# plurigrid/moose

Measured on AMD Instinct MI355X. Metric: replicated fixed(14,23) matmul elems/sec, higher is better.
Workload: dtype fixed(14,23) over Z_2^128 (exact multi-modular int8-MFMA GEMM)

## Files before the change

csrc/gemm_crt.hip:

```cpp
#include <hip/hip_runtime.h>

#include <algorithm>
#include <cmath>
#include <cstdint>
#include <cstdlib>
#include <cstring>
#include <mutex>

#include "hip_attr.h"
#include "moosex.h"
#include "prf_dev.h"
#include "rss_fused.h"

void mx_ws_note(int dev, int64_t want, bool ok);
bool mx_ws_malloc(void** p, int64_t bytes);
void mx_ws_shared_note(void);

namespace {

using u64 = uint64_t;
using u128 = unsigned __int128;
typedef int v4i __attribute__((ext_vector_type(4)));
typedef int v16i __attribute__((ext_vector_type(16)));

// ... 997 lines not shown
      r = r == STG - 1 ? 0 : r + 1;
    }
  }
  asm volatile("s_waitcnt vmcnt(0)" ::: "memory");

  const float pf = ep.pf[mi], rcp = ep.rcp[mi];
  const int t16 = ep.t16[mi];
  int8_t* cr = CR + ((int64_t)g * ntiles + tm * tiles_n + tn) * (int64_t)(BM * BN);
#pragma unroll
  for (int i = 0; i < MI; ++i)
#pragma unroll
    for (int j = 0; j < NJ; ++j) {
      int rr[4];
#pragma unroll
      for (int e = 0; e < 4; ++e)
        rr[e] = centered_mod(acc[i][j][e], pf, rcp, t16);
      const int bi = wr * MI + i, bj = wc * NJ + j;
      *(uint32_t*)(cr + ((bi * (BN / 16) + bj) * 64 + lane) * 4) = pack4(rr[0], rr[1], rr[2], rr[3]);
    }
}

template <class T, int BN>
__global__ void __launch_bounds__(256)
    k_crt_recon16(const int8_t* __restrict__ CR, T* __restrict__ C, int64_t M, int64_t N,
                  int64_t tiles_m, int64_t tiles_n, int accumulate, const RecTab rc) {
  constexpr int NK = sizeof(T) / 2;
  constexpr int kCrTile = BM * BN, NBJ = BN / 16;
  const int64_t ntiles = tiles_m * tiles_n;
  const int64_t total = ntiles * (kCrTile / 4);
  const int64_t b = blockIdx.y;
  const int n = rc.n;
  for (int64_t gt = blockIdx.x * (int64_t)blockDim.x + threadIdx.x; gt < total;
       gt += (int64_t)gridDim.x * blockDim.x) {
    const int lane = (int)(gt & 63);
    const int64_t rest = gt >> 6;
    const int blk = (int)(rest % (16 * NBJ));
    const int64_t tile = rest / (16 * NBJ);
    const int64_t off = tile * kCrTile + (blk * 64 + lane) * 4;
    int acc[4][NK];
    float qs[4];
#pragma unroll
    for (int e = 0; e < 4; ++e) {
      qs[e] = 0.f;
#pragma unroll
      for (int k = 0; k < NK; ++k) acc[e][k] = 0;
    }
    const int8_t* src = CR + b * n * ntiles * (int64_t)kCrTile + off;
    for (int i = 0; i < n; ++i) {
      const uint32_t v = *(const uint32_t*)(src + i * ntiles * (int64_t)kCrTile);
      const float rcp = rc.rcp[i];
      int wk[NK];
#pragma unroll
      for (int k = 0; k < NK; ++k) wk[k] = rc.W[i][k];
#pragma unroll
      for (int e = 0; e < 4; ++e) {
        const int c = (int)(int8_t)((v >> (8 * e)) & 0xff);
        qs[e] = __builtin_fmaf((float)c, rcp, qs[e]);
#pragma unroll
        for (int k = 0; k < NK; ++k) acc[e][k] += __mul24(c, wk[k]);
      }
    }
    const int64_t tm = tile / tiles_n, tn = tile % tiles_n;
    const int bi = blk / NBJ, bj = blk % NBJ;
    const int64_t gcol = tn * BN + bj * 16 + (lane & 15);
    T mw = 0;
#pragma unroll
    for (int k = 0; k < NK; ++k) mw |= (T)rc.Mw[k] << (16 * k);
#pragma unroll
    for (int e = 0; e < 4; ++e) {
      const int64_t grow = tm * BM + bi * 16 + 4 * (lane >> 4) + e;
      T z = 0;
#pragma unroll
      for (int k = 0; k < NK; ++k) z += (T)(int64_t)acc[e][k] << (16 * k);
      const int q = (int)__builtin_rintf(qs[e]);
      z -= (T)(int64_t)q * mw;
      if (grow < M && gcol < N) {
        T* pc = C + (b * M + grow) * N + gcol;
        *pc = accumulate ? (T)(*pc + z) : z;
      }
    }
  }
}

template <class T, int BN>
__global__ void __launch_bounds__(256)
    k_crt_recon16d(const int8_t* __restrict__ CR, T* __restrict__ C, int64_t M, int64_t N,
                   int64_t tiles_m, int64_t tiles_n, int accumulate, const RecTab4 r4, int n,
                   const RecTab rc) {
  constexpr int ND = (int)sizeof(T);
  constexpr int NK = ND / 2;
  constexpr int kCrTile = BM * BN, NBJ = BN / 16;
  const int64_t ntiles = tiles_m * tiles_n;
  const int64_t total = ntiles * (kCrTile / 4);
  const int64_t b = blockIdx.y;
  for (int64_t gt = blockIdx.x * (int64_t)blockDim.x + threadIdx.x; gt < total;
       gt += (int64_t)gridDim.x * blockDim.x) {
    const int lane = (int)(gt & 63);
    const int64_t rest = gt >> 6;
    const int blk = (int)(rest % (16 * NBJ));
    const int64_t tile = rest / (16 * NBJ);
    const int64_t off = tile * kCrTile + (blk * 64 + lane) * 4;
    int acc[4][ND], aq[4][3];
#pragma unroll
    for (int e = 0; e < 4; ++e) {
#pragma unroll
      for (int d = 0; d < ND; ++d) acc[e][d] = 0;
#pragma unroll
      for (int d = 0; d < 3; ++d) aq[e][d] = 0;
    }
    const int8_t* src = CR + b * n * ntiles * (int64_t)kCrTile + off;
    const int64_t pstride = ntiles * (int64_t)kCrTile;
    for (int g = 0; g < r4.groups; ++g) {
      uint32_t v[4];
#pragma unroll
      for (int u = 0; u < 4; ++u)
        v[u] = 4 * g + u < n ? *(const uint32_t*)(src + (4 * g + u) * pstride) : 0u;
      const uint32_t a0 = __builtin_amdgcn_perm(v[1], v[0], 0x05010400u);
      const uint32_t a1 = __builtin_amdgcn_perm(v[1], v[0], 0x07030602u);
      const uint32_t c0 = __builtin_amdgcn_perm(v[3], v[2], 0x05010400u);
      const uint32_t c1 = __builtin_amdgcn_perm(v[3], v[2], 0x07030602u);
      const int t[4] = {(int)__builtin_amdgcn_perm(c0, a0, 0x05040100u),
                        (int)__builtin_amdgcn_perm(c0, a0, 0x07060302u),
                        (int)__builtin_amdgcn_perm(c1, a1, 0x05040100u),
                        (int)__builtin_amdgcn_perm(c1, a1, 0x07060302u)};
#pragma unroll
      for (int d = 0; d < ND; ++d) {
        const int w = (int)r4.wd[g][d];
#pragma unroll
        for (int e = 0; e < 4; ++e) acc[e][d] = __builtin_amdgcn_sdot4(t[e], w, acc[e][d], false);
      }
#pragma unroll
      for (int d = 0; d < 3; ++d) {
        const int w = (int)r4.rd[g][d];
#pragma unroll
        for (int e = 0; e < 4; ++e) aq[e][d] = __builtin_amdgcn_sdot4(t[e], w, aq[e][d], false);
      }
    }
    const int64_t tm = tile / tiles_n, tn = tile % tiles_n;
    const int bi = blk / NBJ, bj = blk % NBJ;
    const int64_t gcol = tn * BN + bj * 16 + (lane & 15);
    T mw = 0;
#pragma unroll
    for (int k = 0; k < NK; ++k) mw |= (T)rc.Mw[k] << (16 * k);
#pragma unroll
    for (int e = 0; e < 4; ++e) {
      const int64_t grow = tm * BM + bi * 16 + 4 * (lane >> 4) + e;
      T z = 0;
#pragma unroll
      for (int k = 0; k < NK; ++k)
        z += (T)(int64_t)(acc[e][2 * k] + acc[e][2 * k + 1] * 256) << (16 * k);
      const int64_t F = (int64_t)aq[e][0] + (int64_t)aq[e][1] * 256 + (int64_t)aq[e][2] * 65536;
      const int64_t q = (F + (1 << 23)) >> 24;
      z -= (T)q * mw;
      if (grow < M && gcol < N) {
        T* pc = C + (b * M + grow) * N + gcol;
        *pc = accumulate ? (T)(*pc + z) : z;
      }
    }
  }
}

inline int64_t round_up(int64_t x, int64_t m) { return (x + m - 1) / m * m; }

int crt_kernel() {
  const char* e = std::getenv("MOOSEX_CRT_KERNEL");
  const int v = e ? std::atoi(e) : 8;
  return v >= 1 && v <= 16 ? v : 8;
}
bool crt_mfma16() { return crt_kernel() >= 4; }
int recon_dot4() {
  static const int v = [] {
    const char* e = std::getenv("MOOSEX_CRT_RECON");
    return e && e[0] == '0' ? 0 : 1;
  }();
  return v;
}

struct CPlan {
  int n, bn;
  int64_t tiles_m, tiles_n, nkb, a_nkb, ra_bytes, rb_bytes, cr_bytes;
};

CPlan make_cplan(int words, int64_t batch, int64_t M, int64_t N, int64_t K, int mode,
                 bool roll = false) {
  CPlan p;
  p.bn = (crt_kernel() == 3 || crt_kernel() == 5) ? 128 : 256;
  const int64_t kprime = mode ? 2 * K : K;
  p.n = moduli_needed(words, kprime);
  p.tiles_m = (M + BM - 1) / BM;
  p.tiles_n = (N + p.bn - 1) / p.bn;
  p.nkb = round_up(kprime, BK) / BK;
  p.a_nkb = roll ? p.nkb / 2 : p.nkb;
  p.ra_bytes = batch * p.n * p.tiles_m * p.a_nkb * (int64_t)kImg;
  p.rb_bytes = batch * p.n * p.tiles_n * p.nkb * (int64_t)(p.bn * BK);
  p.cr_bytes = batch * p.n * p.tiles_m * p.tiles_n * (int64_t)(BM * p.bn);
  return p;
}

int gemm_group_m() {
  const char* e = std::getenv("MOOSEX_CRT_GROUPM");
  const int v = e ? std::atoi(e) : 8;
  return v >= 1 && v <= 64 ? v : 8;
}

bool prep_packed() {
  static const bool v = [] {
    const char* e = std::getenv("MOOSEX_CRT_PACKED");
    return !(e && e[0] == '0');
  }();
  return v;
}

template <class T>
void launch_prep(const CPlan& p, const Tables& tb, bool is_b, int64_t batch, int64_t R,
                 int64_t K, int64_t xs, const T* X0, const T* X1, int mode, int8_t* out,
                 hipStream_t st, int64_t nkb = -1, int64_t nkb_s = -1,
                 const PrepSrcs& src = PrepSrcs()) {
  if (nkb < 0) nkb = p.nkb;
  if (nkb_s < nkb) nkb_s = nkb;
  const int64_t tiles = is_b ? p.tiles_n : p.tiles_m;
  const int rows = is_b ? p.bn : BM;
  const int64_t work = tiles * nkb * (rows * 4);
  const dim3 grid((unsigned)std::min<int64_t>((work + 255) / 256, 16384), (unsigned)batch);
  static const bool packed_b = [] {
    const char* e = std::getenv("MOOSEX_CRT_PACKED_B");
    return e && e[0] == '1';
  }();
  if (!prep_packed() || (is_b && !packed_b)) {
    if (!is_b)
      hipLaunchKernelGGL((k_crt_prep<T, false, BM, false>), grid, dim3(256), 0, st, X0, X1, R, K,
                         xs, mode, out, tiles, nkb, nkb_s, tb.pa, src);
    else if (rows == 256)
      hipLaunchKernelGGL((k_crt_prep<T, true, 256, false>), grid, dim3(256), 0, st, X0, X1, R, K,
                         xs, mode, out, tiles, nkb, nkb_s, tb.pb, src);
    else
      hipLaunchKernelGGL((k_crt_prep<T, true, 128, false>), grid, dim3(256), 0, st, X0, X1, R, K,
                         xs, mode, out, tiles, nkb, nkb_s, tb.pb, src);
    return;
  }
  if (!is_b)
    hipLaunchKernelGGL((k_crt_prep<T, false, BM>), grid, dim3(256), 0, st, X0, X1, R, K, xs, mode,
// ... 51 lines not shown
    hipLaunchKernelGGL((k_crt_prep_src<true, 256, false>), grid, dim3(256), 0, st, s, src.key, R,
                       K, out, tiles, p.a_nkb, tb.pb);
  else
    hipLaunchKernelGGL((k_crt_prep_src<true, 128, false>), grid, dim3(256), 0, st, s, src.key, R,
                       K, out, tiles, p.a_nkb, tb.pb);
}

int dma_mask() {
  const char* e = std::getenv("MOOSEX_CRT_DMA_MASK");
  return e ? std::atoi(e) : 3;
}

template <int WR, int WC, int BN, int MINW, bool M16, int STG = kStages, int IL = 0>
void launch_variant(const CPlan& p, const Tables& tb, int64_t batch, const int8_t* ra,
                    const int8_t* rb, int8_t* cr, int bcast, int roll, hipStream_t st,
                    int amap = 0, int bmap = 0) {
  constexpr int lds = STG * (kImg + BN * BK);
  const void* fn = M16 ? (const void*)k_crt_gemm16<WR, WC, BN, MINW, STG, IL>
                       : (const void*)k_crt_gemm<WR, WC, BN, MINW>;
  ensure_lds_attr(fn, lds, st);
  const dim3 grid((unsigned)(p.tiles_m * p.tiles_n), (unsigned)(batch * p.n));
  if constexpr (M16)
    hipLaunchKernelGGL((k_crt_gemm16<WR, WC, BN, MINW, STG, IL>), grid, dim3(64 * WR * WC), lds, st, ra,
                       rb, cr, (int)p.tiles_m, (int)p.tiles_n, (int)p.nkb, gemm_group_m(), tb.ep,
                       dma_mask(), bcast, (int)p.a_nkb, roll, amap, bmap);
  else
    hipLaunchKernelGGL((k_crt_gemm<WR, WC, BN, MINW>), grid, dim3(64 * WR * WC), lds, st, ra, rb,
                       cr, (int)p.tiles_m, (int)p.tiles_n, (int)p.nkb, gemm_group_m(), tb.ep,
                       dma_mask(), bcast);
}

void launch_crt_gemm(const CPlan& p, const Tables& tb, int64_t batch, const int8_t* ra,
                     const int8_t* rb, int8_t* cr, int bcast, int roll, hipStream_t st,
                     int amap = 0, int bmap = 0) {
  switch (crt_kernel()) {
    case 1: launch_variant<2, 2, 256, 1, false>(p, tb, batch, ra, rb, cr, bcast, 0, st); break;
    case 2: launch_variant<2, 4, 256, 2, false>(p, tb, batch, ra, rb, cr, bcast, 0, st); break;
    case 4: launch_variant<2, 2, 256, 1, true>(p, tb, batch, ra, rb, cr, bcast, roll, st, amap, bmap); break;
    case 3: launch_variant<2, 2, 128, 2, false>(p, tb, batch, ra, rb, cr, bcast, 0, st); break;
    case 6: launch_variant<2, 4, 256, 2, true>(p, tb, batch, ra, rb, cr, bcast, roll, st, amap, bmap); break;
    case 7: launch_variant<2, 4, 256, 2, true, 4>(p, tb, batch, ra, rb, cr, bcast, roll, st, amap, bmap); break;
    case 8: launch_variant<2, 4, 256, 2, true, 3, 1>(p, tb, batch, ra, rb, cr, bcast, roll, st, amap, bmap); break;
    case 9: launch_variant<2, 4, 256, 2, true, 4, 1>(p, tb, batch, ra, rb, cr, bcast, roll, st, amap, bmap); break;
    case 10: launch_variant<2, 4, 256, 2, true, 3, 2>(p, tb, batch, ra, rb, cr, bcast, roll, st, amap, bmap); break;
    case 11: launch_variant<2, 4, 256, 2, true, 4, 2>(p, tb, batch, ra, rb, cr, bcast, roll, st, amap, bmap); break;
    case 12: launch_variant<2, 2, 256, 1, true, 3, 1>(p, tb, batch, ra, rb, cr, bcast, roll, st, amap, bmap); break;
    case 13: launch_variant<2, 2, 256, 1, true, 4, 1>(p, tb, batch, ra, rb, cr, bcast, roll, st, amap, bmap); break;
    case 14: launch_variant<2, 2, 256, 1, true, 3, 2>(p, tb, batch, ra, rb, cr, bcast, roll, st, amap, bmap); break;
    case 15: launch_variant<2, 2, 256, 1, true, 4, 2>(p, tb, batch, ra, rb, cr, bcast, roll, st, amap, bmap); break;
    case 16: launch_variant<2, 4, 256, 2, true, 5, 3>(p, tb, batch, ra, rb, cr, bcast, roll, st, amap, bmap); break;
    default: launch_variant<2, 2, 128, 2, true>(p, tb, batch, ra, rb, cr, bcast, roll, st, amap, bmap); break;
  }
}

template <class T>
void launch_recon(const CPlan& p, const Tables& tb, int64_t batch, int64_t M, int64_t N,
                  const int8_t* cr, T* C, int accumulate, hipStream_t st) {
  const int64_t work = p.tiles_m * p.tiles_n * (BM * p.bn / 8);
  const int gx = (int)std::min<int64_t>((work + 255) / 256, 16384);
  if (crt_mfma16() && recon_dot4()) {
    const int gx16 = (int)std::min<int64_t>((2 * work + 255) / 256, 16384);
    if (p.bn == 256)
      hipLaunchKernelGGL((k_crt_recon16d<T, 256>), dim3(gx16, (unsigned)batch), dim3(256), 0, st,
                         cr, C, M, N, p.tiles_m, p.tiles_n, accumulate, tb.r4, p.n, tb.rc);
    else
      hipLaunchKernelGGL((k_crt_recon16d<T, 128>), dim3(gx16, (unsigned)batch), dim3(256), 0, st,
                         cr, C, M, N, p.tiles_m, p.tiles_n, accumulate, tb.r4, p.n, tb.rc);
  } else if (crt_mfma16()) {
    const int gx16 = (int)std::min<int64_t>((2 * work + 255) / 256, 16384);
    if (p.bn == 256)
      hipLaunchKernelGGL((k_crt_recon16<T, 256>), dim3(gx16, (unsigned)batch), dim3(256), 0, st,
                         cr, C, M, N, p.tiles_m, p.tiles_n, accumulate, tb.rc);
    else
      hipLaunchKernelGGL((k_crt_recon16<T, 128>), dim3(gx16, (unsigned)batch), dim3(256), 0, st,
                         cr, C, M, N, p.tiles_m, p.tiles_n, accumulate, tb.rc);
  } else if (p.bn == 256)
    hipLaunchKernelGGL((k_crt_recon<T, 256>), dim3(gx, (unsigned)batch), dim3(256), 0, st, cr, C,
                       M, N, p.tiles_m, p.tiles_n, accumulate, tb.rc);
  else
    hipLaunchKernelGGL((k_crt_recon<T, 128>), dim3(gx, (unsigned)batch), dim3(256), 0, st, cr, C,
                       M, N, p.tiles_m, p.tiles_n, accumulate, tb.rc);
}

struct Ws {
  void* ptr = nullptr;
  int64_t bytes = 0;
  hipStream_t stream = nullptr;
  bool used = false;
};
std::mutex g_mu;
constexpr int kWsPerDev = 128;
Ws g_ws[16][kWsPerDev];

void* workspace(int64_t bytes, hipStream_t st) {
  int dev = 0;
  hipGetDevice(&dev);
  if (dev < 0 || dev >= 16) return nullptr;
  std::lock_guard<std::mutex> lk(g_mu);
  Ws* slot = nullptr;
  for (int i = 0; i < kWsPerDev && !slot; ++i)
    if (g_ws[dev][i].used && g_ws[dev][i].stream == st) slot = &g_ws[dev][i];
  for (int i = 0; i < kWsPerDev && !slot; ++i)
    if (!g_ws[dev][i].used) {
      slot = &g_ws[dev][i];
      slot->used = true;
      slot->stream = st;
    }
  if (!slot) {
    slot = &g_ws[dev][kWsPerDev - 1];
    mx_ws_shared_note();
  }
  Ws& w = *slot;
  if (w.bytes < bytes) {
    int64_t want = 1 << 20;
    while (want < bytes) want <<= 1;
    void* q = nullptr;
    const bool ok = mx_ws_malloc(&q, want);
    mx_ws_note(dev, want, ok);
    if (!ok) return nullptr;
    w.ptr = q;
    w.bytes = want;
  }
  return w.ptr;
}

template <class T>
int run_crt(int64_t batch, int64_t M, int64_t N, int64_t K, const T* A0, const T* A1,
            int64_t a_bstride, const T* B0, const T* B1, int64_t b_bstride,
            const int8_t* rb_pre, int mode, T* C, int accumulate, hipStream_t st,
            int64_t roll = 0) {
  constexpr int words = sizeof(T) / 8;
  if (roll && (mode != 1 || K % BK || !crt_mfma16() || a_bstride == 0 || batch < 2 ||
               roll % batch == 0))
    return -7;
  const CPlan p = make_cplan(words, batch, M, N, K, mode, roll != 0);
  if (p.n < 0) return -6;
  if ((mode ? 2 * K : K) > (1 << 15)) return -6;
  const Tables& tb = tables_for(words, p.n);
  const int64_t need = p.ra_bytes + (rb_pre ? 0 : p.rb_bytes) + p.cr_bytes;
  int8_t* ws = (int8_t*)workspace(need, st);
  if (!ws) return -4;
  int8_t* ra = ws;
  int8_t* cr = ra + p.ra_bytes;
  const int8_t* rb = rb_pre;
  const bool a_bc = batch > 1 && a_bstride == 0;
  const bool b_bc = batch > 1 && b_bstride == 0 && !rb_pre;
  if (!rb) {
    int8_t* rbw = cr + p.cr_bytes;
    launch_prep<T>(p, tb, true, b_bc ? 1 : batch, N, K, b_bstride, B0, B1, mode, rbw, st);
    rb = rbw;
  }
  if (roll)
    launch_prep<T>(p, tb, false, batch, M, K, a_bstride, A0, A0, 0, ra, st, p.a_nkb);
  else
    launch_prep<T>(p, tb, false, a_bc ? 1 : batch, M, K, a_bstride, A0, A1, mode, ra, st);
  launch_crt_gemm(p, tb, batch, ra, rb, cr, (a_bc ? 1 : 0) | (b_bc ? 2 : 0),
                  (int)(((roll % batch) + batch) % batch), st);
  launch_recon<T>(p, tb, batch, M, N, cr, C, accumulate, st);
  const hipError_t e = hipGetLastError();
  return e != hipSuccess ? -100 - (int)e : 0;
}

template <class T>
int run_crt_asym(int64_t M, int64_t N, int64_t K, const T* S0, const T* S1, const T* T0,
                 const T* T1, int rolled, T* C, hipStream_t st, const ShareSrc* xs = nullptr,
                 const ShareSrc* ys = nullptr) {
  constexpr int words = sizeof(T) / 8;
  if (K % BK || !crt_mfma16()) return -7;
  if (2 * K > (1 << 15)) return -6;
  const CPlan p = make_cplan(words, 3, M, N, K, 1, true);
  if (p.n < 0) return -6;
  const Tables& tb = tables_for(words, p.n);
  const int64_t sa = M * K, sb = K * N;
  const T* a[3];
  const T* b[3];
  const T* c[3];
  const T* d[3];
  for (int q = 0; q < 3; ++q) {
    a[q] = S0 + q * sa;
    b[q] = rolled ? S0 + ((q + 1) % 3) * sa : S1 + q * sa;
    c[q] = T0 + q * sb;
    d[q] = rolled ? T0 + ((q + 1) % 3) * sb : T1 + q * sb;
  }
  int na, nb, amap, bmap;
  const int64_t a_entry = p.n * p.tiles_m * p.a_nkb * (int64_t)kImg;
  const int64_t b_entry = p.n * p.tiles_n * p.a_nkb * (int64_t)(p.bn * BK);
  auto pmap = [](int e0, int e1, int e2, int e3, int e4) {
    return (int)(0x80000000u | (unsigned)e0 | (1u << 6) | ((unsigned)(e1 | (e2 << 3)) << 8) |
                 ((unsigned)(e3 | (e4 << 3)) << 16));
  };
  if (rolled) {
    na = 4;
    nb = 4;
    amap = pmap(0, 1, 2, 1, 3);
    bmap = pmap(0, 1, 2, 3, 2);
  } else {
    na = 5;
    nb = 5;
    amap = pmap(0, 1, 2, 3, 4);
    bmap = pmap(0, 1, 2, 3, 4);
  }
  static const bool asum = [] {
    const char* e = std::getenv("MOOSEX_CRT_ASUM");
    return !(e && e[0] == '0');
  }();
  static const bool dual = [] {
    const char* e = std::getenv("MOOSEX_CRT_DUAL");
    return !(e && e[0] == '0');
  }();
  const bool duals = rolled && dual;
  if (xs || ys) {
    if (words != 2 || !duals) return -7;
    if (xs && (K % 256 || !share_src_ok(*xs))) return -7;
    if (ys && (N % 256 || !share_src_ok(*ys))) return -7;
  }
  static const bool zstrip = [] {
    const char* e = std::getenv("MOOSEX_ZERO_STRIP");
    return !(e && e[0] == '0');
  }();
  int aph[4], bph[4], aat[4] = {0, 1, 2, 3}, bat[4] = {0, 1, 2, 3};
  int64_t a_strip = 0, b_strip = 0;
  auto plan_src = [&](bool is_b, const ShareSrc& s, int (&ph)[4], int (&at)[4], int& n, int& map,
                      int64_t& strip) {
    src_phases(is_b, s, ph);
    int m = 0;
    for (int e = 0; e < 4; ++e) at[e] = zstrip && ph[e] == 3 ? kZeroStrip : m++;
    if (m == n) return;
    n = m;
    strip = p.a_nkb * (int64_t)(is_b ? p.bn * BK : kImg);
    for (int sh : {0, 8, 11, 16, 19}) map = (map & ~(7 << sh)) | (at[(map >> sh) & 7] << sh);
  };
  if (xs) plan_src(false, *xs, aph, aat, na, amap, a_strip);
  if (ys) plan_src(true, *ys, bph, bat, nb, bmap, b_strip);
  const int64_t ra_bytes = na * a_entry, rb_bytes = nb * b_entry;
  const int64_t sum_bytes = asum && !duals ? round_up(sa * (int64_t)sizeof(T), 256) : 0;
  int8_t* ws = (int8_t*)workspace(
      a_strip + ra_bytes + p.cr_bytes + b_strip + rb_bytes + sum_bytes, st);
  if (!ws) return -4;
  int8_t* ra = ws + a_strip;
  int8_t* cr = ra + ra_bytes;
  int8_t* rb = cr + p.cr_bytes + b_strip;
  T* a01 = sum_bytes ? (T*)(rb + rb_bytes) : nullptr;
  if (a01)
    hipLaunchKernelGGL((k_add_pair<T>), dim3((unsigned)std::min<int64_t>((sa + 255) / 256, 65536)),
                       dim3(256), 0, st, a[0], b[0], a01, sa);
  const int64_t kn = p.a_nkb;
  PrepSrcs sa_, sb_;
  auto put = [](PrepSrcs& q, const T* x0, const T* x1, int mode, int64_t dual = 0) {
    q.x0[q.n] = x0;
    q.x1[q.n] = x1;
    q.mode[q.n] = mode;
    q.dual[q.n] = dual;
    ++q.n;
  };
  if (duals) {
    put(sa_, a[2], a[2], 0);
    put(sa_, a[1], a[1], 0);
    put(sa_, a[0], b[0], 0, -3 * a_entry);
    put(sb_, d[1], c[1], 0, -b_entry);
    put(sb_, d[2], d[0], 0, -3 * b_entry);
    if (ys)
      launch_prep_src(p, tb, true, *ys, N, K, rb, b_entry, bph, bat, -b_strip, st);
    else
      launch_prep<T>(p, tb, true, sb_.n, N, K, 0, nullptr, nullptr, 0, rb + 2 * b_entry, st, kn,
                     kn, sb_);
    if (xs)
      launch_prep_src(p, tb, false, *xs, M, K, ra, a_entry, aph, aat, -a_strip, st);
    else
      launch_prep<T>(p, tb, false, sa_.n, M, K, 0, nullptr, nullptr, 0, ra + a_entry, st, kn, kn,
                     sa_);
  } else {
    if (a01)
      put(sa_, a01, a01, 0);
    else
      put(sa_, a[0], b[0], 2);
    put(sb_, c[0], d[0], 3);
    put(sb_, c[1], d[1], 3);
    if (rolled) {
      for (const T* e : {a[2], a[1], a[0]}) put(sa_, e, e, 0);
      for (const T* f : {d[1], d[2]}) put(sb_, f, f, 0);
    } else {
      for (const T* e : {b[1], a[1], a[2], b[2]}) put(sa_, e, e, 0);
      for (const T* f : {d[1], d[2], c[2]}) put(sb_, f, f, 0);
    }
    launch_prep<T>(p, tb, true, sb_.n, N, K, 0, nullptr, nullptr, 0, rb, st, kn, kn, sb_);
    launch_prep<T>(p, tb, false, sa_.n, M, K, 0, nullptr, nullptr, 0, ra, st, kn, kn, sa_);
  }
  launch_crt_gemm(p, tb, 3, ra, rb, cr, 0, 0, st, amap, bmap);
  launch_recon<T>(p, tb, 3, M, N, cr, C, 0, st);
  const hipError_t e = hipGetLastError();
  return e != hipSuccess ? -100 - (int)e : 0;
}

}

extern "C" {

int mx_gemm_asym(int words, int64_t M, int64_t N, int64_t K, const void* S0, const void* S1,
                 const void* T0, const void* T1, int rolled, void* C, void* stream) {
  if (M == 0 || N == 0) return 0;
  if (!rolled && (!S1 || !T1)) return -2;
  hipStream_t st = (hipStream_t)stream;
  if (words == 1)
    return run_crt_asym<u64>(M, N, K, (const u64*)S0, (const u64*)S1, (const u64*)T0,
                             (const u64*)T1, rolled, (u64*)C, st);
  if (words == 2)
    return run_crt_asym<u128>(M, N, K, (const u128*)S0, (const u128*)S1, (const u128*)T0,
                              (const u128*)T1, rolled, (u128*)C, st);
  return -2;
}

int mx_gemm_asym_src(int words, int64_t M, int64_t N, int64_t K, const void* S0, const void* T0,
                     const int64_t* xsrc, const int64_t* ysrc, void* C, void* stream) {
  if (M == 0 || N == 0) return 0;
  if (words != 2) return -7;
  if ((!xsrc && !S0) || (!ysrc && !T0)) return -2;
  ShareSrc sx, sy;
  auto fill = [](ShareSrc& s, const int64_t* a) {
    s.x = (const void*)(intptr_t)a[0];
    s.kind = (int)a[1];
    s.frac = (int)a[2];
    s.j0 = (int)a[3];
    const uint32_t* slot[1] = {(const uint32_t*)(intptr_t)a[4]};
    s.key = mxd::keysrc_slots(slot, 1);
    s.nonce = (uint64_t)a[5];
  };
  if (xsrc) fill(sx, xsrc);
  if (ysrc) fill(sy, ysrc);
  if ((xsrc && !sx.key.slot[0]) || (ysrc && !sy.key.slot[0])) return -2;
  return run_crt_asym<u128>(M, N, K, (const u128*)S0, nullptr, (const u128*)T0, nullptr, 1,
                            (u128*)C, (hipStream_t)stream, xsrc ? &sx : nullptr,
                            ysrc ? &sy : nullptr);
}

int mx_crt_moduli(int words, int64_t kprime) {
  if (words != 1 && words != 2) return -2;
  return moduli_needed(words, kprime);
}

int mx_crt_tables(int words, int n, int32_t* p_out, uint8_t* wa_out, uint8_t* wb_out,
                  int32_t* nega_out, int32_t* negb_out, uint16_t* W_out, uint16_t* Mw_out) {
  if ((words != 1 && words != 2) || n < 1 || n > kMaxMod) return -2;
  const Tables& t = tables_for(words, n);
  for (int i = 0; i < n; ++i) {
    p_out[i] = t.ep.p[i];
    for (int j = 0; j < 16; ++j) {
      wa_out[i * 16 + j] = (uint8_t)(t.pa.w[i][j / 4] >> (8 * (j % 4)));
      wb_out[i * 16 + j] = (uint8_t)(t.pb.w[i][j / 4] >> (8 * (j % 4)));
    }
    nega_out[i] = (int32_t)t.pa.neg[i];
    negb_out[i] = (int32_t)t.pb.neg[i];
    if (i == 0) {
      nega_out[0] = (int32_t)t.pa.mul0;
      negb_out[0] = 1;
    }
    for (int k = 0; k < 8; ++k) W_out[i * 8 + k] = t.rc.W[i][k];
  }
  for (int k = 0; k < 8; ++k) Mw_out[k] = t.rc.Mw[k];
  return 0;
}

int mx_crt_tables4(int words, int n, uint32_t* wd_out, uint32_t* rd_out) {
  if ((words != 1 && words != 2) || n < 1 || n > kMaxMod) return -2;
  const Tables& t = tables_for(words, n);
  for (int g = 0; g < t.r4.groups; ++g) {
    for (int d = 0; d < 16; ++d) wd_out[g * 16 + d] = t.r4.wd[g][d];
    for (int d = 0; d < 3; ++d) rd_out[g * 3 + d] = t.r4.rd[g][d];
  }
  return t.r4.groups;
}

int mx_crt_combine(int words, int n, int side, int i, int64_t count, const int32_t* ra,
                   const int32_t* rb, const int32_t* kappa, int8_t* out) {
  if ((words != 1 && words != 2) || n < 1 || n > kMaxMod || i < 0 || i >= n || (side & ~1))
    return -2;
  const Tables& t = tables_for(words, n);
  const PrepTab& tab = side ? t.pb : t.pa;
  const float p = (float)tab.p[i], rcp = tab.rcp[i];
  for (int64_t k = 0; k < count; ++k) {
    if (side) {
      out[k] = (int8_t)crt_combine(ra[k], rb[k], kappa[k], tab.neg[i], p, rcp);
    } else {
      const f2 f = crt_combine2((f2){(float)ra[k], 0.f}, (f2){(float)rb[k], 0.f},
                                (f2){(float)kappa[k], 0.f}, (float)tab.neg[i], p, rcp);
      out[k] = (int8_t)(int)f.x;
    }
  }
  return 0;
}

int mxh_gemm_crt(int words, int64_t batch, int64_t M, int64_t N, int64_t K, const void* A0,
                 const void* A1, const void* B0, const void* B1, int mode, void* C,
                 int accumulate, void* stream) {
  hipStream_t st = (hipStream_t)stream;
  if (words == 1)
    return run_crt<u64>(batch, M, N, K, (const u64*)A0, (const u64*)A1, M * K, (const u64*)B0,
                        (const u64*)B1, K * N, nullptr, mode, (u64*)C, accumulate, st);
  if (words == 2)
    return run_crt<u128>(batch, M, N, K, (const u128*)A0, (const u128*)A1, M * K,
                         (const u128*)B0, (const u128*)B1, K * N, nullptr, mode, (u128*)C,
                         accumulate, st);
  return -2;
}

int mxh_gemm_crt_strided(int words, int64_t batch, int64_t M, int64_t N, int64_t K,
                         const void* A0, const void* A1, int64_t a_bstride, const void* B0,
                         const void* B1, int64_t b_bstride, int mode, void* C, int accumulate,
                         void* stream) {
  hipStream_t st = (hipStream_t)stream;
  if (words == 1)
    return run_crt<u64>(batch, M, N, K, (const u64*)A0, (const u64*)A1, a_bstride,
                        (const u64*)B0, (const u64*)B1, b_bstride, nullptr, mode, (u64*)C,
                        accumulate, st);
  if (words == 2)
    return run_crt<u128>(batch, M, N, K, (const u128*)A0, (const u128*)A1, a_bstride,
// ... 59 lines not shown
```

csrc/moosex.h:

```cpp
#pragma once
#include <stdint.h>

#ifdef __cplusplus
extern "C" {
#endif

enum mx_binop { MX_ADD = 0, MX_SUB = 1, MX_MUL = 2, MX_AND = 3, MX_OR = 4, MX_XOR = 5 };
enum mx_unop { MX_NEG = 0, MX_NOT = 1, MX_SHL = 2, MX_SHR = 3, MX_SAR = 4 };
enum mx_cmpop { MX_LT = 0, MX_GT = 1, MX_EQ = 2, MX_MSB = 3 };
enum mx_cross { MX_CROSS_ARITH = 0, MX_CROSS_BOOL = 1 };
enum mx_share_src { MX_SHARE_F64 = 2, MX_SHARE_MIRROR = 8 };

typedef struct {
  uint32_t rk[44];
} mx_aes_key;

int mx_version(void);
int mx_device_count(void);

int mx_ew_binary(int dev, int op, int words, const void* a, int64_t na, const void* b,
                 int64_t nb, void* out, int64_t n, void* stream);
int mx_ew_binary_slot(int dev, int op, int words, const void* a, const void* b, int64_t nb,
                      void* out, int64_t m, int nparties, int which, void* stream);
int mx_add_zs3(int dev, int words, const void* v, const void* r, void* out0, void* out1,
               int64_t n, void* stream);
int mx_ew_unary(int dev, int op, int words, const void* a, void* out, int64_t n,
                int64_t param, void* stream);
int mx_ew_binary2(int dev, int op, int words, const void* a0, const void* b0, void* out0,
                  const void* a1, const void* b1, void* out1, int64_t na, int64_t nb, int64_t n,
                  void* stream);
int mx_mul_add2(int dev, int words, const void* a0, const void* a1, const void* f,
                const void* c, int add0, int add1, void* out0, void* out1, int64_t n,
                void* stream);
int mx_ew_unary2(int dev, int op, int words, const void* a0, void* out0, const void* a1,
                 void* out1, int64_t n, int64_t param, void* stream);
int mx_transpose2(int dev, int words, const void* a0, void* out0, const void* a1, void* out1,
                  int64_t rows, int64_t cols, void* stream);
int mx_im2col(int dev, int elem_bytes, const void* in, void* out, int64_t slots,
              int64_t in_slot_stride, int64_t N, int64_t C, int64_t H, int64_t W, int64_t KH,
              int64_t KW, int64_t sh, int64_t sw, int64_t pt, int64_t pl, int64_t dh,
              int64_t dw, int64_t OH, int64_t OW, int nhwc, void* stream);
int mx_col2im(int dev, int elem_bytes, const void* in, void* out, int64_t slots,
              int64_t in_slot_stride, int64_t N, int64_t C, int64_t H, int64_t W, int64_t KH,
              int64_t KW, int64_t sh, int64_t sw, int64_t pt, int64_t pl, int64_t dh,
              int64_t dw, int64_t OH, int64_t OW, int nhwc, void* stream);
int mx_resize2d(int dev, int elem_bytes, const void* in, void* out, int64_t slots,
                int64_t in_slot_stride, int64_t N, int64_t C, int64_t H, int64_t W, int64_t OH,
                int64_t OW, const int32_t* th, const int32_t* tw, int wbh, int wbw, int nhwc,
                void* stream);
int mx_dwconv(int dev, int elem_bytes, const void* x0, const void* x1, const void* w0,
              const void* w1, void* out, int64_t slots, int64_t x_slot_stride,
              int64_t w_slot_stride, int64_t N, int64_t C, int64_t H, int64_t W, int64_t mult,
              int64_t KH, int64_t KW, int64_t sh, int64_t sw, int64_t pt, int64_t pl,
              int64_t dh, int64_t dw, int64_t OH, int64_t OW, int nhwc, void* stream);
#define MX_PWL_MAX 8
int mx_pwl_cross(int dev, int elem_bytes, const void* s0, const void* s1, const void* x0,
                 const void* x1, void* out, int64_t slots, int64_t s_slot_stride,
                 int64_t x_slot_stride, int64_t n, int k, const uint64_t* da, const uint64_t* db,
                 const uint64_t* ak, void* stream);
int mx_ew_binary_slot2(int dev, int op, int words, const void* a0, const void* a1,
                       const void* b, int64_t nb, void* out0, void* out1, int64_t m,
                       int nparties, int which0, int which1, void* stream);
int mx_mul_trunc3_kv(int dev, int words, const void* x0, const void* x1, const void* y0,
                     const void* y1, void* out0, void* out1, int64_t n, int64_t ostride,
                     const uint32_t* slots, uint64_t nmul, int m, const uint64_t* nonces,
                     const int64_t* views, void* stream);
int mx_mul_trunc3_open(int dev, int words, const void* x, int64_t xstride, double* out,
                       int64_t n, const uint32_t* slots, uint64_t nmul, int m,
                       const uint64_t* nonces, int frac, void* stream);
int mx_ew_add3(int dev, int words, const void* a, const void* b, const void* c, void* out,
               int64_t n, void* stream);
int mx_lincomb2(int dev, int words, int nin, const void* const* ins, const int64_t* coef,
                const void* b, int64_t nb, void* out0, void* out1, int64_t m, int nparties,
                int which0, int which1, void* stream);
int mx_sum_views2(int dev, int words, const void* base0, const void* base1, int64_t is0,
                  int64_t is1, int64_t ps0, int64_t ps1, int k, void* out0, void* out1, int64_t m,
                  int nparties, void* stream);
int mx_slot_place2(int dev, int words, const void* x0, const void* x1, void* out0, void* out1,
                   int64_t m, int nparties, int which0, int which1, void* stream);
int mx_ew_compare(int dev, int op, int words, const void* a, int64_t na, const void* b,
                  int64_t nb, uint8_t* out, int64_t n, void* stream);
int mx_bit_extract(int dev, int words, const void* a, uint8_t* out, int64_t n, int bit,
                   void* stream);
int mx_ring_inject(int dev, int words, const uint8_t* bits, void* out, int64_t n, int bit,
                   void* stream);
int mx_encode(int dev, int words, const double* x, void* out, int64_t n, int frac,
              void* stream);
int mx_addn_decode(int dev, int words, const void* a, const void* b, const void* c,
                   const void* d, double* out, int64_t n, int frac, void* stream);
int mx_decode(int dev, int words, const void* x, double* out, int64_t n, int frac,
              void* stream);
int mx_fill(int dev, int words, void* out, int64_t n, uint64_t lo, uint64_t hi, void* stream);
int mx_bit_planes(int dev, int words, const void* a, uint8_t* out, int64_t outer, int64_t inner,
                  int start, int count, void* stream);
int mx_weighted_sum(int dev, int words, const void* a, const void* w, void* out, int64_t outer,
                    int64_t k, int64_t inner, void* stream);
int mx_sum_axis(int dev, int words, const void* a, void* out, int64_t outer, int64_t red,
                int64_t inner, void* stream);
int mx_prg(int dev, const uint8_t* key16, uint64_t nonce, uint64_t ctr0, void* out,
           int64_t nbytes, void* stream);
int mx_derive_seed(const uint8_t* key16, const uint8_t* sync16, uint8_t* out16);
int mx_aes_encrypt_blocks(const uint8_t* key16, const uint8_t* in, uint8_t* out,
                          int64_t nblocks);
int mx_rss_cross(int dev, int kind, int words, const void* x0, const void* x1,
                 const void* y0, const void* y1, void* out, int64_t n, int nparties,
                 const uint8_t* keys16, uint64_t nonce, void* stream);
int mx_zero_share(int dev, int kind, int words, void* out, int64_t n, int nparties,
                  const uint8_t* keys16, uint64_t nonce, void* stream);
int mx_prf_expand(int dev, int words, void* out, int64_t n, int nkeys,
                  const uint8_t* keys16, uint64_t nonce, void* stream);
int mx_gemm(int dev, int words, int64_t batch, int64_t M, int64_t N, int64_t K,
            const void* A0, const void* A1, const void* B0, const void* B1, int mode,
            void* C, int accumulate, void* stream);
int64_t mx_gemm_workspace_bytes(int words, int64_t batch, int64_t M, int64_t N,
                                int64_t K, int mode);
int64_t mx_workspace_failed_bytes(void);
int64_t mx_workspace_held_bytes(void);
int64_t mx_workspace_shared_count(void);
int mx_gemm_ws(int words, int64_t batch, int64_t M, int64_t N, int64_t K, const void* A0,
               const void* A1, const void* B0, const void* B1, int mode, void* C,
               int accumulate, void* workspace, int64_t ws_bytes, void* stream);
int64_t mx_gemm_b_bytes(int words, int64_t batch, int64_t N, int64_t K, int mode);
int mx_gemm_prep_b(int words, int64_t batch, int64_t K, int64_t N, const void* B0,
                   const void* B1, int mode, void* lb, void* stream);
int mx_gemm_with_b(int words, int64_t batch, int64_t M, int64_t N, int64_t K, const void* A0,
                   const void* A1, int64_t a_bstride, int mode, const void* lb, void* C,
                   int accumulate, void* stream);
int mx_crt_tables4(int words, int n, uint32_t* wd_out, uint32_t* rd_out);
int mx_gemm_roll(int words, int64_t batch, int64_t M, int64_t N, int64_t K, const void* A0,
                 int64_t a_bstride, int64_t roll, const void* B0, const void* B1, const void* lb,
                 void* C, int accumulate, void* stream);
int mx_gemm_strided(int words, int64_t batch, int64_t M, int64_t N, int64_t K, const void* A0,
                    const void* A1, int64_t a_bstride, const void* B0, const void* B1,
                    int64_t b_bstride, int mode, void* C, int accumulate, void* stream);
void mx_set_gemm_impl(int impl);
void mx_set_gemm_crt(int mode);
int mx_crt_moduli(int words, int64_t kprime);
int mx_crt_tables(int words, int n, int32_t* p, uint8_t* wa, uint8_t* wb, int32_t* nega,
                  int32_t* negb, uint16_t* W, uint16_t* Mw);
int mx_crt_combine(int words, int n, int side, int i, int64_t count, const int32_t* ra,
                   const int32_t* rb, const int32_t* kappa, int8_t* out);

int mx_trunc_pr3(int dev, int words, const void* s0, void* out0, void* out1, int64_t n, int m,
                 const uint8_t* k0, const uint8_t* k2, const uint64_t* nonces, void* stream);
int mx_share3(int dev, int kind, int words, const void* x, void* out0, void* out1, int64_t n,
              int j, const uint8_t* k_next, const uint8_t* k_all, uint64_t n1, uint64_t na,
              void* stream);

#define MX_KEY_SLOT_WORDS 48
void mx_key_slots(const uint8_t* keys16, int n, uint32_t* out);
int mx_rss_cross_k(int dev, int kind, int words, const void* x0, const void* x1,
                   const void* y0, const void* y1, void* out, int64_t n, int nparties,
// ... 112 lines not shown
```

csrc/ring_common.h:

```cpp
#pragma once
#include <stdint.h>
#include <string.h>

#include "aes_core.h"
#include "img_geom.h"
#include "moosex.h"

namespace mxr {

using u64 = uint64_t;
using u128 = unsigned __int128;
using i128 = __int128;

template <class T>
struct Bits {
  static constexpr int value = 8 * sizeof(T);
};

template <class T>
MX_HD inline T binop(int op, T a, T b) {
  if constexpr (sizeof(T) == 1) {
    switch (op) {
      case MX_ADD:
      case MX_SUB:
// ... 64 lines not shown
    }
  } else {
    i128 x = (i128)a, y = (i128)b;
    switch (op) {
      case MX_LT: return x < y;
      case MX_GT: return x > y;
      case MX_EQ: return x == y;
      default: return (uint8_t)(a >> 127);
    }
  }
}

template <class T>
MX_HD inline T cross(int kind, T x0, T x1, T y0, T y1, bool has_x1, bool has_y1) {
  if (kind == MX_CROSS_BOOL) {
    T v = x0 & y0;
    if (has_y1) v ^= x0 & y1;
    if (has_x1) v ^= x1 & y0;
    return v;
  }
  T v = x0 * y0;
  if (has_y1) v += x0 * y1;
  if (has_x1) v += x1 * y0;
  return v;
}

template <class T>
MX_HD inline T zs_combine(int kind, T v, T ra, T rb) {
  if (kind == MX_CROSS_BOOL) return (T)(v ^ ra ^ rb);
  return (T)(v + ra - rb);
}


MX_HD inline i128 f64_to_i128(double x) {
  uint64_t bits;
  memcpy(&bits, &x, 8);
  int neg = (int)(bits >> 63);
  int e = (int)((bits >> 52) & 0x7ff);
  uint64_t mant = bits & ((1ull << 52) - 1);
  if (e == 0x7ff) return mant ? (i128)0 : (neg ? (i128)((u128)1 << 127) : ~(i128)((u128)1 << 127));
  if (e == 0) return 0;
  mant |= (1ull << 52);
  int sh = e - 1075;
  u128 mag;
  if (sh >= 0) {
    if (sh > 127 - 53) return neg ? (i128)((u128)1 << 127) : ~(i128)((u128)1 << 127);
    mag = (u128)mant << sh;
  } else if (sh <= -53) {
    mag = 0;
  } else {
    mag = (u128)(mant >> (-sh));
  }
  return neg ? -(i128)mag : (i128)mag;
}

template <class T>
MX_HD inline T f64_to_ring(double x) {
  if constexpr (sizeof(T) == 8) {
    if (x >= 9223372036854775808.0) return (T)0x7fffffffffffffffull;
    if (x > -9223372036854775808.0) return (T)(int64_t)x;
    return x != x ? (T)0 : (T)1 << 63;
  } else {
    return (T)f64_to_i128(x);
  }
}

MX_HD inline double i128_to_f64(u128 v) {
  const bool neg = (v >> 127) != 0;
  const u128 m = neg ? (u128)0 - v : v;
  const uint64_t hi = (uint64_t)(m >> 64), lo = (uint64_t)m;
  double r;
  if (hi == 0) {
    r = (double)lo;
  } else {
    const int s = 64 - __builtin_clzll(hi);
    const uint64_t lost = s == 64 ? lo : lo & ((1ull << s) - 1);
    const uint64_t top = (uint64_t)(m >> s) | (uint64_t)(lost != 0);
    const uint64_t pbits = (uint64_t)(1023 + s) << 52;
    double p;
    memcpy(&p, &pbits, 8);
    r = (double)top * p;
  }
  return neg ? -r : r;
}

}

extern "C" {
int mxh_ew_binary(int op, int words, const void* a, int64_t na, const void* b, int64_t nb,
                  void* out, int64_t n, void* stream);
int mxh_ew_unary(int op, int words, const void* a, void* out, int64_t n, int64_t param,
                 void* stream);
int mxh_ew_compare(int op, int words, const void* a, int64_t na, const void* b, int64_t nb,
                   uint8_t* out, int64_t n, void* stream);
int mxh_bit_extract(int words, const void* a, uint8_t* out, int64_t n, int bit, void* stream);
int mxh_ring_inject(int words, const uint8_t* bits, void* out, int64_t n, int bit,
                    void* stream);
int mxh_encode(int words, const double* x, void* out, int64_t n, int frac, void* stream);
int mxh_decode(int words, const void* x, double* out, int64_t n, int frac, void* stream);
int mxh_addn_decode(int words, const void* a, const void* b, const void* c, const void* d,
                    double* out, int64_t n, int frac, void* stream);
int mxh_fill(int words, void* out, int64_t n, uint64_t lo, uint64_t hi, void* stream);
int mxh_bit_planes(int words, const void* a, uint8_t* out, int64_t outer, int64_t inner,
                   int start, int count, void* stream);
int mxh_weighted_sum(int words, const void* a, const void* w, void* out, int64_t outer,
                     int64_t k, int64_t inner, void* stream);
int mxh_sum_axis(int words, const void* a, void* out, int64_t outer, int64_t red, int64_t inner,
                 void* stream);
int mxh_prg(const uint8_t* key16, uint64_t nonce, uint64_t ctr0, void* out, int64_t nbytes,
            void* stream);
int mxh_rss_cross(int kind, int words, const void* x0, const void* x1, const void* y0,
                  const void* y1, void* out, int64_t n, int nparties, const uint8_t* keys16,
                  uint64_t nonce, void* stream);
int mxh_prf_expand(int words, void* out, int64_t n, int nkeys, const uint8_t* keys16,
                   uint64_t nonce, void* stream);
int mxh_rss_cross_kp(int kind, int words, const void* x0, const void* x1, const void* y0,
                     const void* y1, void* out, int64_t n, int nparties,
                     const uint32_t* const* slot_ptrs, uint64_t nonce, void* stream);
int mxh_rss_cross_k(int kind, int words, const void* x0, const void* x1, const void* y0,
                    const void* y1, void* out, int64_t n, int nparties, const uint32_t* slots,
                    int nslots, uint64_t nonce, void* stream);
int mxh_rss_mul3_kv(int kind, int words, const void* x0, const void* x1, const void* y0,
                    const void* y1, void* out0, void* out1, int64_t n, const uint32_t* slots,
                    uint64_t nonce, const int64_t* views, void* stream);
int mxh_rss_mul3_k(int kind, int words, const void* x0, const void* x1, const void* y0,
                   const void* y1, void* out0, void* out1, int64_t n, const uint32_t* slots,
                   uint64_t nonce, void* stream);
int mxh_ew_binary_slot(int op, int words, const void* a, const void* b, int64_t nb, void* out,
                       int64_t m, int nparties, int which, void* stream);
int mxh_add_zs3(int words, const void* v, const void* r, void* out0, void* out1, int64_t n,
                void* stream);
int mxh_ew_binary2(int op, int words, const void* a0, const void* b0, void* out0,
                   const void* a1, const void* b1, void* out1, int64_t na, int64_t nb, int64_t n,
                   void* stream);
int mxh_mul_add2(int words, const void* a0, const void* a1, const void* f, const void* c,
                 int add0, int add1, void* out0, void* out1, int64_t n, void* stream);
int mxh_ew_add3(int words, const void* a, const void* b, const void* c, void* out, int64_t n,
                void* stream);
int mxh_lincomb2(int words, int nin, const void* const* ins, const int64_t* coef, const void* b,
                 int64_t nb, void* out0, void* out1, int64_t m, int nparties, int which0,
                 int which1, void* stream);
int mxh_sum_views2(int words, const void* base0, const void* base1, int64_t is0, int64_t is1,
                   int64_t ps0, int64_t ps1, int k, void* out0, void* out1, int64_t m,
                   int nparties, void* stream);
int mxh_slot_place2(int words, const void* x0, const void* x1, void* out0, void* out1,
                    int64_t m, int nparties, int which0, int which1, void* stream);
int mxh_mul_trunc3_kv(int words, const void* x0, const void* x1, const void* y0, const void* y1,
                      void* out0, void* out1, int64_t n, int64_t ostride, const uint32_t* slots,
                      uint64_t nmul, int m, const uint64_t* nn, const int64_t* views,
                      void* stream);
int mxh_mul_trunc3_open(int words, const void* x, int64_t xstride, double* out, int64_t n,
                        const uint32_t* slots, uint64_t nmul, int m, const uint64_t* nn, int frac,
                        void* stream);
int mxh_ew_unary2(int op, int words, const void* a0, void* out0, const void* a1, void* out1,
                  int64_t n, int64_t param, void* stream);
int mxh_transpose2(int words, const void* a0, void* out0, const void* a1, void* out1,
                   int64_t rows, int64_t cols, void* stream);
int mxh_ew_binary_slot2(int op, int words, const void* a0, const void* a1, const void* b,
                        int64_t nb, void* out0, void* out1, int64_t m, int nparties, int which0,
                        int which1, void* stream);
int mxh_im2col(int elem_bytes, const void* in, void* out, int64_t slots, int64_t in_slot_stride,
               const mxr::ImgGeom& g, void* stream);
int mxh_col2im(int elem_bytes, const void* in, void* out, int64_t slots, int64_t in_slot_stride,
               const mxr::ImgGeom& g, void* stream);
int mxh_resize2d(int elem_bytes, const void* in, void* out, int64_t slots,
                 int64_t in_slot_stride, const mxr::ImgGeom& g, const int32_t* th,
                 const int32_t* tw, void* stream);
int mxh_pwl_cross(int elem_bytes, const void* s0, const void* s1, const void* x0, const void* x1,
                  void* out, int64_t slots, int64_t s_slot_stride, int64_t x_slot_stride,
                  int64_t n, int k, const uint64_t* da, const uint64_t* db, const uint64_t* ak,
                  void* stream);
int mxh_dwconv(int elem_bytes, const void* x0, const void* x1, const void* w0, const void* w1,
               void* out, int64_t slots, int64_t x_slot_stride, int64_t w_slot_stride,
               const mxr::ImgGeom& g, void* stream);
int mxh_ks_cross1(int words, const void* g0, const void* g1, const void* p0, const void* p1,
                  void* z, int64_t n, int d, int both, const uint8_t* keys16, uint64_t nonce,
                  void* stream);
int mxh_ks_cross1_s(int words, const void* g0, const void* g1, const void* p0, const void* p1,
                    void* z, int64_t n, int d, int both, const uint32_t* const* slots,
                    uint64_t nonce, void* stream);
int mxh_ks_cross1x_s(int words, const void* g0, const void* g1, const void* t0, const void* t1,
                     void* go0, void* go1, const void* p0, const void* p1, void* z, int64_t n,
                     int d, int both, const uint32_t* const* slots, uint64_t nonce,
                     void* stream);
int mxh_ks_sum2(int words, const void* p0, const void* p1, const void* g0, const void* g1,
                const void* t0, const void* t1, void* o0, void* o1, int64_t n, void* stream);
int mxh_ks_adder3_k(int words, const void* g0, const void* g1, const void* p0, const void* p1,
                    void* og0, void* og1, int64_t n, int nlev, const uint32_t* slots,
                    const uint64_t* nonces, void* stream);
int mxh_ks_level3_k(int words, const void* g0, const void* g1, const void* p0, const void* p1,
                    void* og0, void* og1, void* op0, void* op1, int64_t n, int d, int both,
                    const uint32_t* slots, uint64_t nonce, void* stream);
int mxh_prf_expand_k(int words, void* out, int64_t n, int nkeys, const uint32_t* slots,
                     uint64_t nonce, void* stream);
int mxh_gemm(int words, int64_t batch, int64_t M, int64_t N, int64_t K, const void* A0,
             const void* A1, const void* B0, const void* B1, int mode, void* C, int accumulate,
             void* stream);
}
```

csrc/ring_hip.hip:

```cpp
#include <hip/hip_runtime.h>

#include <algorithm>
#include <cstring>
#include <type_traits>

#include "prf_dev.h"
#include "moosex.h"
#include "party_batch.h"
#include "ring_common.h"
#include "rss_fused.h"

using mxr::u128;
using u64 = uint64_t;

namespace {

constexpr int kBlock = 256;

inline int grid_for(int64_t n, int per_thread = 1) {
  int64_t blocks = (n + (int64_t)kBlock * per_thread - 1) / ((int64_t)kBlock * per_thread);
  return (int)std::max<int64_t>(1, std::min<int64_t>(blocks, 256 * 8));
}

inline hipStream_t S(void* s) { return (hipStream_t)s; }
// ... 1308 lines not shown
                                                             const T* __restrict__ y0,
                                                             const T* __restrict__ y1,
                                                             T* __restrict__ out,
                                                             T* __restrict__ out1, int64_t n,
                                                             KeySrc keys, uint64_t nonce, Views vw) {
  constexpr int EPB = 256 / 3;
  __shared__ uint32_t rks[3][kKeyWords];
  __shared__ uint64_t kl[3][EPB], kh[3][EPB];
  stage_keys(rks, keys, 3);
  constexpr int P = Lane<T>::kPer;
  const int64_t nb = (n + P - 1) / P;
  const int tid = threadIdx.x, s = tid / EPB, lb = tid % EPB;
  for (int64_t b0 = (int64_t)blockIdx.x * EPB; b0 < nb; b0 += (int64_t)gridDim.x * EPB) {
    const bool fin = tid < EPB && b0 + tid < nb;
    T vv[3][P];
#pragma unroll
    for (int p = 0; p < 3; ++p) {
#pragma unroll
      for (int j = 0; j < P; ++j) {
        const int64_t e = (b0 + tid) * P + j;
        T v = 0;
        if (fin && e < n) {
          if (x0 != nullptr && y0 != nullptr)
            v = mxr::cross<T>(kind, ld_view(x0, vw, 0, p, e, n),
                              x1 ? ld_view(x1, vw, 1, p, e, n) : (T)0, ld_view(y0, vw, 2, p, e, n),
                              y1 ? ld_view(y1, vw, 3, p, e, n) : (T)0, x1 != nullptr, y1 != nullptr);
          else if (x0 != nullptr)
            v = ld_view(x0, vw, 0, p, e, n);
        }
        vv[p][j] = v;
      }
    }
    if (s < 3 && b0 + lb < nb) {
      uint64_t lo, hi;
      prf_chunk(rks[s], nonce, (uint64_t)(b0 + lb), &lo, &hi);
      kl[s][lb] = lo;
      kh[s][lb] = hi;
    }
    __syncthreads();
    if (fin) {
      const int64_t b = b0 + tid;
#pragma unroll
      for (int p = 0; p < 3; ++p) {
        const int q = p == 2 ? 0 : p + 1;
#pragma unroll
        for (int j = 0; j < P; ++j) {
          const int64_t e = b * P + j;
          if (e >= n) break;
          const int64_t i = (int64_t)p * n + e;
          const T v = vv[p][j];
          const T z = mxr::zs_combine<T>(kind, v, pick<T>(kl[p][tid], kh[p][tid], j),
                                         pick<T>(kl[q][tid], kh[q][tid], j));
          out[i] = z;
          if (out1 != nullptr) out1[(int64_t)(p == 0 ? 2 : p - 1) * n + e] = z;
        }
      }
    }
    __syncthreads();
  }
}

template <class T>
struct TailShares {
  T* __restrict__ out0;
  T* __restrict__ out1;
  int64_t os;
  __device__ __forceinline__ void operator()(int64_t e, T Z0, T Z1, T Z2) const {
    out0[e] = Z0;
    out0[os + e] = Z1;
    out0[2 * os + e] = Z2;
    if (out1 != out0 + os) {
      out1[e] = Z1;
      out1[os + e] = Z2;
    }
    out1[2 * os + e] = Z0;
  }
};

template <class T>
struct TailOpen {
  double* __restrict__ out;
  double scale;
  __device__ __forceinline__ void operator()(int64_t e, T Z0, T Z1, T Z2) const {
    const T v = Z0 + Z1 + Z2;
    if constexpr (sizeof(T) == 8)
      out[e] = (double)(int64_t)v * scale;
    else
      out[e] = mxr::i128_to_f64(v) * scale;
  }
};

template <class T, int EPB, class Sink>
__device__ __forceinline__ void mul_trunc3_lat_body(
    const T* __restrict__ x0, const T* __restrict__ x1, const T* __restrict__ y0,
    const T* __restrict__ y1, const Sink& sink, int64_t n,
    const uint32_t (&rks)[3][kKeyWords], uint64_t (&kl)[9][EPB], uint64_t (&kh)[9][EPB],
    uint64_t nmul, int m, uint64_t nr0, uint64_t nr1, uint64_t nt, uint64_t nm, uint64_t nz0,
    uint64_t nz2, const Views& vw) {
  constexpr int NS = 9;
  constexpr int P = Lane<T>::kPer;
  const int64_t nb = (n + P - 1) / P;
  const int tid = threadIdx.x, s = tid / EPB, lb = tid % EPB;
  const int key_of = s < 3 ? s : (s == 4 || s == 8) ? 2 : 0;
  const uint64_t nonce_of = s < 3 ? nmul : s == 3 ? nr0 : s == 4 ? nr1 : s == 5 ? nt
                            : s == 6 ? nm : s == 7 ? nz0 : nz2;
  for (int64_t b0 = (int64_t)blockIdx.x * EPB; b0 < nb; b0 += (int64_t)gridDim.x * EPB) {
    const bool fin = tid < EPB && b0 + tid < nb;
    T vv[P][3];
#pragma unroll
    for (int j = 0; j < P; ++j) {
      const int64_t e = (b0 + tid) * P + j;
#pragma unroll
      for (int p = 0; p < 3; ++p)
        vv[j][p] = !fin || e >= n ? (T)0
                   : y0 == nullptr ? ld_view(x0, vw, 0, p, e, n)
                   : mxr::cross<T>(MX_CROSS_ARITH, ld_view(x0, vw, 0, p, e, n),
                                   ld_view(x1, vw, 1, p, e, n), ld_view(y0, vw, 2, p, e, n),
                                   ld_view(y1, vw, 3, p, e, n), true, true);
    }
    if (s < NS && b0 + lb < nb) {
      uint64_t lo, hi;
      prf_chunk(rks[key_of], nonce_of, (uint64_t)(b0 + lb), &lo, &hi);
      kl[s][lb] = lo;
      kh[s][lb] = hi;
    }
    __syncthreads();
    if (fin) {
      const int64_t b = b0 + tid;
#pragma unroll
      for (int j = 0; j < P; ++j) {
        const int64_t e = b * P + j;
        if (e >= n) break;
        T z[3];
#pragma unroll
        for (int p = 0; p < 3; ++p) {
          const int q = p == 2 ? 0 : p + 1;
          z[p] = mxr::zs_combine<T>(MX_CROSS_ARITH, vv[j][p], pick<T>(kl[p][tid], kh[p][tid], j),
                                    pick<T>(kl[q][tid], kh[q][tid], j));
        }
        const T Z0 = pick<T>(kl[7][tid], kh[7][tid], j);
        const T Z2 = pick<T>(kl[8][tid], kh[8][tid], j);
        const T Z1 = mxf::trunc_pr_z1<T>(
            z[0], z[1], z[2], pick<T>(kl[3][tid], kh[3][tid], j),
            pick<T>(kl[4][tid], kh[4][tid], j), pick<T>(kl[5][tid], kh[5][tid], j),
            pick<T>(kl[6][tid], kh[6][tid], j), Z0, Z2, m);
        sink(e, Z0, Z1, Z2);
      }
    }
    __syncthreads();
  }
}

template <class T>
__global__ void __launch_bounds__(256) k_mul_trunc3_lat(
    const T* __restrict__ x0, const T* __restrict__ x1, const T* __restrict__ y0,
    const T* __restrict__ y1, T* __restrict__ out0, T* __restrict__ out1, int64_t n, int64_t os,
    KeySrc keys, uint64_t nmul, int m, uint64_t nr0, uint64_t nr1, uint64_t nt, uint64_t nm,
    uint64_t nz0, uint64_t nz2, Views vw) {
  constexpr int EPB = 256 / 9;
  __shared__ uint32_t rks[3][kKeyWords];
  __shared__ uint64_t kl[9][EPB], kh[9][EPB];
  stage_keys(rks, keys, 3);
  mul_trunc3_lat_body<T, EPB>(x0, x1, y0, y1, TailShares<T>{out0, out1, os}, n, rks, kl, kh,
                              nmul, m, nr0, nr1, nt, nm, nz0, nz2, vw);
}

template <class T>
__global__ void __launch_bounds__(256) k_mul_trunc3_lat_open(
    const T* __restrict__ x, double* __restrict__ out, double scale, int64_t n, KeySrc keys,
    uint64_t nmul, int m, uint64_t nr0, uint64_t nr1, uint64_t nt, uint64_t nm, uint64_t nz0,
    uint64_t nz2, Views vw) {
// ... 1805 lines not shown
```

csrc/rss_fused.h:

```cpp
#pragma once
#include <stdint.h>

#include "aes_core.h"
#include "moosex.h"
#include "ring_common.h"

namespace mxf {

template <class T>
MX_HD inline T shl(T x, int k) {
  constexpr int W = 8 * sizeof(T);
  return k >= W ? (T)0 : (T)(x << k);
}
template <class T>
MX_HD inline T shr(T x, int k) {
  constexpr int W = 8 * sizeof(T);
  return k >= W ? (T)0 : (T)(x >> k);
}

template <class T>
MX_HD inline T trunc_pr_z1(T x0, T x1, T x2, T r0, T r1, T rt0, T rm0, T z0, T z2, int m) {
  constexpr int W = 8 * sizeof(T);
  const int k = W - 1;
  T r = r0 + r1;
  T r_msb = shr<T>(r, W - 1);
  T r_top = shr<T>(shl<T>(r, 1), m + 1);
  T rt1 = r_top - rt0;
  T rm1 = r_msb - rm0;
  T mk0 = x0 + x1 + shl<T>((T)1, k - 1) + r0;
  T mk1 = x2 + r1;
  T c = mk0 + mk1;
  T c_msb = shr<T>(c, W - 1);
  T c_top = shr<T>(shl<T>(c, 1), m + 1);
  T ov0 = rm0 - shl<T>(c_msb * rm0, 1) + c_msb;
  T y0 = shl<T>(ov0, k - m) - rt0 + c_top - shl<T>((T)1, k - 1 - m);
  T ov1 = rm1 - shl<T>(c_msb * rm1, 1);
  T y1 = shl<T>(ov1, k - m) - rt1;
  return (y0 - z0) + (y1 - z2);
}

template <class T>
MX_HD inline T share_plain(int kind, const void* xv, int64_t i, double scale) {
  return kind == MX_SHARE_F64 ? mxr::f64_to_ring<T>(((const double*)xv)[i] * scale)
                              : ((const T*)xv)[i];
}
template <class T>
MX_HD inline T share_masked(int kind, T x, T r) {
  return kind == MX_CROSS_BOOL ? (T)(x ^ r) : (T)(x - r);
}
MX_HD inline void share_place(int j0, bool mir, int* jr, int* jv) {
  *jr = mir ? (j0 + 1) % 3 : j0;
  *jv = mir ? j0 : (j0 + 1) % 3;
}
template <class T>
MX_HD inline void share_slots(int kind, T x, T r, int j0, bool mir, T (&slot)[3]) {
  const T v = share_masked<T>(kind, x, r);
  slot[j0] = mir ? v : r;
  slot[(j0 + 1) % 3] = mir ? r : v;
  slot[(j0 + 2) % 3] = 0;
}

using u128_t = unsigned __int128;

constexpr int64_t kRingExtendLatMax = 8192;

MX_HD inline void ring_extend_dealer(uint64_t r0, uint64_t r1, u128_t R0, uint64_t M0, u128_t* R1,
                                     uint64_t* M1) {
  const uint64_t r = r0 + r1;
  *R1 = (u128_t)r - R0;
  *M1 = (r >> 63) - M0;
}

MX_HD inline uint64_t ring_extend_mask0(uint64_t x0, uint64_t x1, uint64_t r0) {
  return x0 + x1 + ((uint64_t)1 << 62) + r0;
}

MX_HD inline u128_t ring_extend_y(uint64_t c, u128_t R, uint64_t M, bool first) {
  const uint64_t nc = 1 - (c >> 63);
  const u128_t y = ((u128_t)(uint64_t)(nc * M) << 64) - R;
  return first ? y + (u128_t)c - ((u128_t)1 << 62) : y;
}

MX_HD inline u128_t ring_extend_z1(uint64_t x0, uint64_t x1, uint64_t x2, uint64_t r0, uint64_t r1,
                                   u128_t R0, uint64_t M0, u128_t z0, u128_t z2) {
  u128_t R1;
  uint64_t M1;
  ring_extend_dealer(r0, r1, R0, M0, &R1, &M1);
  const uint64_t c = ring_extend_mask0(x0, x1, r0) + (x2 + r1);
  const u128_t y0 = ring_extend_y(c, R0, M0, true);
  const u128_t y1 = ring_extend_y(c, R1, M1, false);
  return (y0 - z0) + (y1 - z2);
}

}

namespace mxf {

template <class T>
MX_HD inline void trunc_dealer(T r0, T r1, T rt0, T rm0, int m, T* rt1, uint64_t* rm1) {
  constexpr int W = 8 * sizeof(T);
  const T r = r0 + r1;
  *rt1 = shr<T>(shl<T>(r, 1), m + 1) - rt0;
  *rm1 = (uint64_t)(shr<T>(r, W - 1) - rm0);
}

template <class T>
MX_HD inline T trunc_mask0(T x0, T x1, T r0) {
  constexpr int W = 8 * sizeof(T);
  return x0 + x1 + shl<T>((T)1, W - 2) + r0;
}

template <class T>
MX_HD inline T trunc_y(T c, T rt, T rm, int m, bool first) {
  constexpr int W = 8 * sizeof(T);
  const int k = W - 1;
  const T c_msb = shr<T>(c, W - 1);
  T ov = rm - shl<T>(c_msb * rm, 1);
  if (!first) return shl<T>(ov, k - m) - rt;
  ov = ov + c_msb;
  const T c_top = shr<T>(shl<T>(c, 1), m + 1);
  return shl<T>(ov, k - m) - rt + c_top - shl<T>((T)1, k - 1 - m);
// ... 52 lines not shown
```

csrc/rss_fused_cpu.cpp:

```cpp
#include <cmath>
#include <cstring>
#include <functional>
#include <vector>

#include "moosex.h"
#include "ring_common.h"
#include "rss_fused.h"

void mx_cpu_prf_range(const uint8_t* key, uint64_t nonce, int words, int64_t i0, int64_t n,
                      void* out);
void mx_cpu_parallel_for(int64_t n, int64_t grain,
                         const std::function<void(int64_t, int64_t)>& f);

extern "C" int mxh_trunc_pr3(int words, const void* s0, void* out0, void* out1, int64_t n, int m,
                             const uint8_t* k0, const uint8_t* k2, const uint64_t* nonces,
                             void* stream);
extern "C" int mxh_share3(int kind, int words, const void* x, void* out0, void* out1, int64_t n,
                          int j, const uint8_t* k_next, const uint8_t* k_all, uint64_t n1,
                          uint64_t na, void* stream);
extern "C" int mxh_trunc_pr3_k(int words, const void* s0, void* out0, void* out1, int64_t n,
                               int m, const uint32_t* slot_k0, const uint32_t* slot_k2,
                               const uint64_t* nonces, void* stream);
extern "C" int mxh_trunc_pr3_kmo(int words, const void* s0, void* out0, void* out1, int64_t n,
                                 int m, const uint32_t* slot_k0, const uint32_t* slot_k2,
// ... 144 lines not shown
                 const uint8_t* k0, const uint8_t* k2, const uint64_t* nonces, void* stream) {
  if (dev) return mxh_trunc_pr3(words, s0, out0, out1, n, m, k0, k2, nonces, stream);
  if (words == 1)
    return trunc3_host<uint64_t>((const uint64_t*)s0, (uint64_t*)out0, (uint64_t*)out1, n, m, k0,
                                 k2, nonces);
  if (words == 2)
    return trunc3_host<unsigned __int128>((const unsigned __int128*)s0, (unsigned __int128*)out0,
                                          (unsigned __int128*)out1, n, m, k0, k2, nonces);
  return -2;
}

int mx_share3(int dev, int kind, int words, const void* x, void* out0, void* out1, int64_t n,
              int j, const uint8_t* k_next, const uint8_t* k_all, uint64_t n1, uint64_t na,
              void* stream) {
  if (dev) return mxh_share3(kind, words, x, out0, out1, n, j, k_next, k_all, n1, na, stream);
  switch (words) {
    case 0:
      return share3_host<uint8_t>(kind, (const uint8_t*)x, (uint8_t*)out0, (uint8_t*)out1, n, j,
                                  k_next, k_all, n1, na);
    case 1:
      return share3_host<uint64_t>(kind, (const uint64_t*)x, (uint64_t*)out0, (uint64_t*)out1, n,
                                   j, k_next, k_all, n1, na);
    case 2:
      return share3_host<unsigned __int128>(kind, (const unsigned __int128*)x,
                                            (unsigned __int128*)out0, (unsigned __int128*)out1, n,
                                            j, k_next, k_all, n1, na);
  }
  return -2;
}

int mx_trunc_pr3_k(int dev, int words, const void* s0, void* out0, void* out1, int64_t n, int m,
                   const uint32_t* slot_k0, const uint32_t* slot_k2, const uint64_t* nonces,
                   void* stream) {
  if (dev)
    return mxh_trunc_pr3_k(words, s0, out0, out1, n, m, slot_k0, slot_k2, nonces, stream);
  return mx_trunc_pr3(0, words, s0, out0, out1, n, m, (const uint8_t*)slot_k0,
                      (const uint8_t*)slot_k2, nonces, stream);
}

int mx_trunc_pr3_ko(int dev, int words, const void* s0, void* out0, void* out1, int64_t n,
                    int m, const uint32_t* slot_k0, const uint32_t* slot_k2,
                    const uint64_t* nonces, int64_t ostride, void* stream) {
  if (dev)
    return mxh_trunc_pr3_ko(words, s0, out0, out1, n, m, slot_k0, slot_k2, nonces, ostride,
                            stream);
  if (words != 1 && words != 2) return -2;
  const size_t es = 8 * (size_t)words;
  std::vector<uint8_t> t0(3 * n * es), t1(3 * n * es);
  int rc = mx_trunc_pr3_k(0, words, s0, t0.data(), t1.data(), n, m, slot_k0, slot_k2, nonces,
                          stream);
  if (rc) return rc;
  for (int p = 0; p < 3; ++p) {
    std::memcpy((uint8_t*)out0 + p * ostride * es, t0.data() + p * n * es, n * es);
    std::memcpy((uint8_t*)out1 + p * ostride * es, t1.data() + p * n * es, n * es);
  }
  return 0;
}

int mx_trunc_pr3_kmo(int dev, int words, const void* s0, void* out0, void* out1, int64_t n,
                     int m, const uint32_t* slot_k0, const uint32_t* slot_k2,
                     const uint64_t* nonces, int64_t ostride, const uint64_t* cm, void* stream) {
  if (dev)
    return mxh_trunc_pr3_kmo(words, s0, out0, out1, n, m, slot_k0, slot_k2, nonces, ostride, cm,
                             stream);
  if (words == 1) {
    std::vector<uint64_t> t(3 * n);
    for (int64_t i = 0; i < 3 * n; ++i) t[i] = ((const uint64_t*)s0)[i] * cm[0];
    return mx_trunc_pr3_ko(0, words, t.data(), out0, out1, n, m, slot_k0, slot_k2, nonces,
                           ostride, stream);
  }
  if (words == 2) {
    using u128 = unsigned __int128;
    const u128 c = ((u128)cm[1] << 64) | cm[0];
    std::vector<u128> t(3 * n);
    for (int64_t i = 0; i < 3 * n; ++i) t[i] = ((const u128*)s0)[i] * c;
    return mx_trunc_pr3_ko(0, words, t.data(), out0, out1, n, m, slot_k0, slot_k2, nonces,
                           ostride, stream);
  }
  return -2;
}

int mx_mul_trunc3_open(int dev, int words, const void* x, int64_t xstride, double* out,
                       int64_t n, const uint32_t* slots, uint64_t nmul, int m,
                       const uint64_t* nonces, int frac, void* stream) {
  if (words != 1 && words != 2) return -2;
  if (m < 1 || m > 63) return -3;
  if (dev) return mxh_mul_trunc3_open(words, x, xstride, out, n, slots, nmul, m, nonces, frac,
                                      stream);
  if (xstride < n) return -3;
  const uint8_t* k[3];
  for (int i = 0; i < 3; ++i) k[i] = (const uint8_t*)(slots + MX_KEY_SLOT_WORDS * i);
  if (words == 1)
    return mul_trunc3_open_host<uint64_t>((const uint64_t*)x, xstride, out, n, k, nmul, m,
                                          nonces, frac);
  return mul_trunc3_open_host<unsigned __int128>((const unsigned __int128*)x, xstride, out, n, k,
                                                 nmul, m, nonces, frac);
}

int mx_ring_extend3_k(int dev, const void* s0, void* out0, void* out1, int64_t n,
                      const uint32_t* slot_k0, const uint32_t* slot_k2, const uint64_t* nonces,
                      void* stream) {
  if (dev) return mxh_ring_extend3_k(s0, out0, out1, n, slot_k0, slot_k2, nonces, stream);
  return ring_extend3_host((const uint64_t*)s0, (unsigned __int128*)out0,
                           (unsigned __int128*)out1, n, (const uint8_t*)slot_k0,
                           (const uint8_t*)slot_k2, nonces);
}

int64_t mx_ring_extend3_lat_max(void) { return mxf::kRingExtendLatMax; }

int mx_share3_k(int dev, int kind, int words, const void* x, void* out0, void* out1, int64_t n,
                int j, const uint32_t* slot_next, const uint32_t* slot_all, uint64_t n1,
                uint64_t na, void* stream) {
  if (dev)
    return mxh_share3_k(kind, words, x, out0, out1, n, j, slot_next, slot_all, n1, na, stream);
  return mx_share3(0, kind, words, x, out0, out1, n, j, (const uint8_t*)slot_next,
                   (const uint8_t*)slot_all, n1, na, stream);
}

}
```

moose_amd/ops/native.py:

```python
from __future__ import annotations

import ctypes
import os
import threading

import torch

from moose_amd import errors
from moose_amd._native import build as _build

_LIB = None
_LOCK = threading.Lock()

c_i64 = ctypes.c_int64
c_int = ctypes.c_int
c_u64 = ctypes.c_uint64
c_vp = ctypes.c_void_p

_SIGS = {
    "mx_version": (c_int, []),
    "mx_device_count": (c_int, []),
    "mx_ew_binary": (c_int, [c_int, c_int, c_int, c_vp, c_i64, c_vp, c_i64, c_vp, c_i64, c_vp]),
    "mx_ew_unary": (c_int, [c_int, c_int, c_int, c_vp, c_vp, c_i64, c_i64, c_vp]),
    "mx_mul_add2": (c_int, [c_int, c_int, c_vp, c_vp, c_vp, c_vp, c_int, c_int, c_vp, c_vp,
                            c_i64, c_vp]),
    "mx_ew_binary2": (c_int, [c_int, c_int, c_int, c_vp, c_vp, c_vp, c_vp, c_vp, c_vp, c_i64,
                              c_i64, c_i64, c_vp]),
    "mx_ew_unary2": (c_int, [c_int, c_int, c_int, c_vp, c_vp, c_vp, c_vp, c_i64, c_i64, c_vp]),
    "mx_transpose2": (c_int, [c_int, c_int, c_vp, c_vp, c_vp, c_vp, c_i64, c_i64, c_vp]),
    "mx_im2col": (c_int, [c_int, c_int, c_vp, c_vp, c_i64, c_i64] + [c_i64] * 14 + [c_int, c_vp]),
    "mx_col2im": (c_int, [c_int, c_int, c_vp, c_vp, c_i64, c_i64] + [c_i64] * 14 + [c_int, c_vp]),
    "mx_resize2d": (c_int, [c_int, c_int, c_vp, c_vp, c_i64, c_i64] + [c_i64] * 6
                    + [c_vp, c_vp, c_int, c_int, c_int, c_vp]),
    "mx_pwl_cross": (c_int, [c_int, c_int] + [c_vp] * 5 + [c_i64] * 4 + [c_int] + [c_vp] * 3
                     + [c_vp]),
    "mx_dwconv": (c_int, [c_int, c_int] + [c_vp] * 5 + [c_i64] * 3 + [c_i64] * 15
                  + [c_int, c_vp]),
    "mx_ew_binary_slot2": (c_int, [c_int, c_int, c_int, c_vp, c_vp, c_vp, c_i64, c_vp, c_vp,
                                   c_i64, c_int, c_int, c_int, c_vp]),
    "mx_mul_trunc3_kv": (c_int, [c_int, c_int, c_vp, c_vp, c_vp, c_vp, c_vp, c_vp, c_i64, c_i64,
                                 c_vp, c_u64, c_int, c_vp, c_vp, c_vp]),
    "mx_mul_trunc3_open": (c_int, [c_int, c_int, c_vp, c_i64, c_vp, c_i64, c_vp, c_u64, c_int,
                                   c_vp, c_int, c_vp]),
    "mx_ew_add3": (c_int, [c_int, c_int, c_vp, c_vp, c_vp, c_vp, c_i64, c_vp]),
    "mx_lincomb2": (c_int, [c_int, c_int, c_int, c_vp, c_vp, c_vp, c_i64, c_vp, c_vp, c_i64,
                            c_int, c_int, c_int, c_vp]),
    "mx_sum_views2": (c_int, [c_int, c_int, c_vp, c_vp, c_i64, c_i64, c_i64, c_i64, c_int, c_vp,
                              c_vp, c_i64, c_int, c_vp]),
    "mx_slot_place2": (c_int, [c_int, c_int, c_vp, c_vp, c_vp, c_vp, c_i64, c_int, c_int, c_int,
                               c_vp]),
    "mx_ew_compare": (c_int, [c_int, c_int, c_int, c_vp, c_i64, c_vp, c_i64, c_vp, c_i64, c_vp]),
    "mx_bit_extract": (c_int, [c_int, c_int, c_vp, c_vp, c_i64, c_int, c_vp]),
    "mx_ring_inject": (c_int, [c_int, c_int, c_vp, c_vp, c_i64, c_int, c_vp]),
    "mx_encode": (c_int, [c_int, c_int, c_vp, c_vp, c_i64, c_int, c_vp]),
    "mx_decode": (c_int, [c_int, c_int, c_vp, c_vp, c_i64, c_int, c_vp]),
    "mx_addn_decode": (c_int, [c_int, c_int, c_vp, c_vp, c_vp, c_vp, c_vp, c_i64, c_int, c_vp]),
    "mx_sum_axis": (c_int, [c_int, c_int, c_vp, c_vp, c_i64, c_i64, c_i64, c_vp]),
    "mx_fill": (c_int, [c_int, c_int, c_vp, c_i64, c_u64, c_u64, c_vp]),
    "mx_bit_planes": (c_int, [c_int, c_int, c_vp, c_vp, c_i64, c_i64, c_int, c_int, c_vp]),
    "mx_weighted_sum": (c_int, [c_int, c_int, c_vp, c_vp, c_vp, c_i64, c_i64, c_i64, c_vp]),
    "mx_prg": (c_int, [c_int, c_vp, c_u64, c_u64, c_vp, c_i64, c_vp]),
    "mx_aes_encrypt_blocks": (c_int, [c_vp, c_vp, c_vp, c_i64]),
    "mx_derive_seed": (c_int, [c_vp, c_vp, c_vp]),
    "mx_rss_cross": (
        c_int,
        [c_int, c_int, c_int, c_vp, c_vp, c_vp, c_vp, c_vp, c_i64, c_int, c_vp, c_u64, c_vp],
    ),
    "mx_zero_share": (c_int, [c_int, c_int, c_int, c_vp, c_i64, c_int, c_vp, c_u64, c_vp]),
    "mx_prf_expand": (c_int, [c_int, c_int, c_vp, c_i64, c_int, c_vp, c_u64, c_vp]),
    "mx_gemm": (
        c_int,
        [c_int, c_int, c_i64, c_i64, c_i64, c_i64, c_vp, c_vp, c_vp, c_vp, c_int, c_vp, c_int, c_vp],
    ),
    "mx_gemm_workspace_bytes": (c_i64, [c_int, c_i64, c_i64, c_i64, c_i64, c_int]),
    "mx_workspace_failed_bytes": (c_i64, []),
    "mx_workspace_held_bytes": (c_i64, []),
    "mx_workspace_shared_count": (c_i64, []),
    "mx_mfma_peak": (c_int, [c_int, c_int, c_vp, c_vp]),
    "mx_gemm_ws": (
        c_int,
        [c_int, c_i64, c_i64, c_i64, c_i64, c_vp, c_vp, c_vp, c_vp, c_int, c_vp, c_int, c_vp,
         c_i64, c_vp],
    ),
    "mx_set_gemm_impl": (None, [c_int]),
    "mx_set_gemm_crt": (None, [c_int]),
    "mx_gemm_strided": (
        c_int,
        [c_int, c_i64, c_i64, c_i64, c_i64, c_vp, c_vp, c_i64, c_vp, c_vp, c_i64, c_int, c_vp,
         c_int, c_vp],
    ),
    "mxh_wsum_trunc3": (
        c_int, [c_int, c_vp, c_i64, c_i64, c_int, c_vp, c_vp, c_vp, c_i64, c_int, c_vp, c_vp,
                c_vp, c_vp, c_vp],
    ),
    "mxh_mul_trunc3_kv2": (
        c_int, [c_int, c_vp, c_vp, c_vp, c_vp, c_vp, c_vp, c_vp, c_vp, c_vp, c_vp, c_vp, c_vp,
                c_vp, c_vp],
    ),
    "mxh_b2a_prep3": (c_int, [c_int, c_vp, c_vp, c_i64, c_vp, c_vp, c_vp, c_vp]),
    "mxh_b2a3_planes": (
        c_int, [c_int, c_vp, c_vp, c_i64, c_int, c_int, c_vp, c_vp, c_vp, c_int, c_u64, c_u64,
                c_vp],
    ),
    "mxh_mul_rows_add": (c_int, [c_int, c_vp, c_vp, c_vp, c_i64, c_i64, c_vp, c_int, c_int, c_vp]),
    "mxh_mux3": (
        c_int, [c_int, c_vp, c_vp, c_vp, c_vp, c_vp, c_vp, c_vp, c_vp, c_i64, c_vp, c_u64, c_int,
                c_vp],
    ),
    "mxh_bitdec3": (
        c_int, [c_int, c_vp, c_vp, c_vp, c_vp, c_i64, c_int, c_vp, c_int, c_u64, c_u64, c_vp,
                c_int, c_u64, c_u64, c_vp],
    ),
    "mxh_b2a3": (
        c_int, [c_int, c_vp, c_vp, c_i64, c_vp, c_vp, c_vp, c_int, c_u64, c_u64, c_vp],
    ),
    "mxh_gemm_bs": (
        c_int, [c_int, c_i64, c_i64, c_i64, c_i64, c_vp, c_i64, c_vp, c_i64, c_vp, c_vp],
    ),
    "mx_crt_moduli": (c_int, [c_int, c_i64]),
    "mx_crt_tables": (c_int, [c_int, c_int, c_vp, c_vp, c_vp, c_vp, c_vp, c_vp, c_vp]),
    "mx_trunc_pr3": (
        c_int, [c_int, c_int, c_vp, c_vp, c_vp, c_i64, c_int, c_vp, c_vp, c_vp, c_vp],
    ),
    "mx_key_slots": (None, [ctypes.c_char_p, c_int, c_vp]),
    "mx_rss_cross_k": (
        c_int,
# ... 60 lines not shown
        [c_int, c_int, c_int, c_vp, c_vp, c_vp, c_i64, c_int, c_vp, c_vp, c_u64, c_u64, c_vp],
    ),
    "mx_ring_extend3_k": (c_int, [c_int, c_vp, c_vp, c_vp, c_i64, c_vp, c_vp, c_vp, c_vp]),
    "mx_ring_extend3_lat_max": (c_i64, []),
    "mx_trunc_party_r0": (
        c_int,
        [c_int, c_int, c_i64, c_int, c_int, c_vp, c_vp, c_vp, c_vp, c_vp, c_vp, c_vp, c_vp,
         c_vp, c_vp],
    ),
    "mx_trunc_party_r1": (
        c_int,
        [c_int, c_int, c_i64, c_int, c_int, c_vp, c_vp, c_vp, c_vp, c_vp, c_vp, c_vp, c_vp,
         c_vp, c_vp, c_vp],
    ),
    "mx_ring_extend_party_r0": (
        c_int,
        [c_int, c_i64, c_int, c_vp, c_vp, c_vp, c_vp, c_vp, c_vp, c_vp, c_vp, c_vp, c_vp, c_vp],
    ),
    "mx_ring_extend_party_r1": (
        c_int,
        [c_int, c_i64, c_int, c_vp, c_vp, c_vp, c_vp, c_vp, c_vp, c_vp, c_vp, c_vp, c_vp, c_vp],
    ),
    "mx_dot_tail_r0": (
        c_int,
        [c_int, c_int, c_i64, c_int, c_int, c_vp, c_vp, c_vp, c_vp, c_vp, c_vp, c_vp, c_vp,
         c_vp, c_vp],
    ),
    "mx_dot_tail_r1": (
        c_int,
        [c_int, c_int, c_i64, c_int, c_int, c_vp, c_vp, c_vp, c_vp, c_vp, c_vp, c_vp, c_vp,
         c_vp, c_vp, c_vp, c_vp],
    ),
    "mx_dot_tail_r2": (c_int, [c_int, c_int, c_i64, c_int, c_vp, c_vp, c_vp, c_vp, c_vp]),
    "mx_share_party": (
        c_int,
        [c_int, c_int, c_int, c_i64, c_int, c_vp, c_vp, c_vp, c_vp, c_vp, c_u64, c_u64, c_vp],
    ),
    "mx_gemm_b_bytes": (c_i64, [c_int, c_i64, c_i64, c_i64, c_int]),
    "mx_gemm_prep_b": (c_int, [c_int, c_i64, c_i64, c_i64, c_vp, c_vp, c_int, c_vp, c_vp]),
    "mx_gemm_with_b": (
        c_int,
        [c_int, c_i64, c_i64, c_i64, c_i64, c_vp, c_vp, c_i64, c_int, c_vp, c_vp, c_int, c_vp],
    ),
    "mx_share3": (
        c_int,
        [c_int, c_int, c_int, c_vp, c_vp, c_vp, c_i64, c_int, c_vp, c_vp, c_u64, c_u64, c_vp],
    ),
    "mx_crt_tables4": (c_int, [c_int, c_int, c_vp, c_vp]),
    "mx_crt_combine": (c_int, [c_int, c_int, c_int, c_int, c_i64, c_vp, c_vp, c_vp, c_vp]),
    "mx_copy_channels": (c_int, [c_vp, c_vp, c_i64, c_int, c_vp]),
    "mx_stream_cumask": (c_int, [c_vp, c_int, c_vp]),
    "mx_stream_destroy": (c_int, [c_vp]),
    "mx_graph_compose": (c_int, [c_int, c_vp, c_vp, c_vp, c_vp, c_vp, c_vp, c_vp, c_vp, c_vp]),
    "mx_graph_compose_merged": (c_int, [c_int, c_vp, c_vp, c_vp, c_vp, c_vp, c_vp, c_vp, c_vp,
                                        c_vp]),
    "mx_graph_dot": (c_int, [c_vp, ctypes.c_char_p, ctypes.c_uint]),
    "mx_graph_launch": (c_int, [c_vp, c_vp]),
    "mx_enable_peer": (c_int, [c_int, c_int]),
    "mx_alloc_uncached": (c_int, [c_int, c_i64, c_vp]),
    "mx_free_uncached": (c_int, [c_int, c_vp]),
    "mx_graph_build_chain": (c_int, [c_int, c_vp, c_vp, c_vp, c_vp, c_vp, c_vp, c_vp, c_vp,
                                     c_vp]),
    "mx_jobs_r0": (c_int, [c_int, c_int, c_int, c_vp, c_vp, c_i64, c_int, c_int, c_int, c_int,
                           c_vp, c_vp, c_vp, c_vp, c_vp, c_vp]),
    "mx_jobs_r0p": (c_int, [c_int, c_int, c_int, c_vp, c_vp, c_i64, c_int, c_int, c_int, c_int,
                            c_vp, c_vp, c_vp, c_vp, c_vp, c_int, c_vp, c_vp, c_vp]),
    "mx_jobs_r1": (c_int, [c_int, c_int, c_int, c_vp, c_vp, c_i64, c_int, c_int, c_vp, c_vp, c_vp,
                           c_vp, c_vp, c_vp, c_vp, c_vp, c_vp]),
    "mx_jobs_r2": (c_int, [c_int, c_int, c_int, c_vp, c_vp, c_i64, c_int, c_vp, c_vp, c_vp]),
    "mx_bits_front": (c_int, [c_int, c_int, c_int, c_i64, c_vp, c_vp, c_vp, c_vp, c_vp, c_vp,
                              c_vp, c_vp, c_vp, c_vp]),
    "mx_wsum_pair": (c_int, [c_int, c_int, c_int, c_int, c_int, c_int, c_int, c_i64, c_i64,
                             c_vp, c_vp, c_vp, c_vp, c_vp, c_vp, c_vp, c_vp, c_vp, c_vp, c_vp,
                             c_vp, c_vp, c_vp]),
    "mx_bits_b2a": (c_int, [c_int, c_int, c_int, c_int, c_i64, c_int, c_int, c_int, c_int,
                            c_vp, c_vp, c_vp,
                            c_vp, c_vp, c_vp, c_vp, c_vp, c_vp, c_vp, c_vp, c_vp]),
    "mx_key_refresh": (c_int, [c_vp, c_int, c_vp, c_vp, c_vp]),
    "mx_copy_async": (c_int, [c_vp, c_vp, ctypes.c_int64, c_vp]),
    "mx_key_refresh_host": (None, [c_vp, c_u64, c_int, c_vp]),
    "mx_copy_many": (c_int, [c_vp, c_int, c_i64, c_vp]),
    "mx_graph_free": (c_int, [c_vp, c_vp]),
    "mx_gemm_asym": (
        c_int, [c_int, c_i64, c_i64, c_i64, c_vp, c_vp, c_vp, c_vp, c_int, c_vp, c_vp],
    ),
    "mx_gemm_asym_src": (
        c_int, [c_int, c_i64, c_i64, c_i64, c_vp, c_vp, c_vp, c_vp, c_vp, c_vp],
    ),
    "mx_gemm_roll": (
        c_int,
        [c_int, c_i64, c_i64, c_i64, c_i64, c_vp, c_i64, c_i64, c_vp, c_vp, c_vp, c_vp, c_int,
         c_vp],
    ),
}


class NativeError(errors.KernelError):
    pass


def lib():
    global _LIB
    if _LIB is not None:
        return _LIB
    with _LOCK:
        if _LIB is not None:
            return _LIB
        if _build.needs_build() and os.environ.get("MOOSEX_NO_BUILD") != "1":
            _build.build()
        path = os.environ.get("MOOSEX_LIB") or str(_build.LIB)
        try:
            handle = ctypes.CDLL(path, mode=ctypes.RTLD_GLOBAL)
        except OSError as e:
            raise NativeError(f"cannot load {path}: {e}") from e
        for name, (res, args) in _SIGS.items():
            fn = getattr(handle, name)
            fn.restype = res
            fn.argtypes = args
        _LIB = handle
        return _LIB


def loaded_path():
    return str(_build.LIB)


def check(rc, what):
    if rc != 0:
        if rc == -4:
            raise NativeError(workspace_error(what, _ws_failed_bytes(), _ws_held_bytes()))
        raise NativeError(f"{what} failed with code {rc}")


def _ws_failed_bytes() -> int:
    try:
        return int(lib().mx_workspace_failed_bytes())
    except Exception:
        return 0


def _ws_held_bytes() -> int:
    try:
        return int(lib().mx_workspace_held_bytes())
    except Exception:
        return 0


def workspace_error(what: str, failed: int, held: int) -> str:
    gib = 1 << 30
    size = f"{failed / gib:.2f} GiB" if failed else "an unknown size"
    return (f"{what} failed with code -4: the device workspace allocation of {size} "
            f"({failed} bytes) failed; {held / gib:.2f} GiB of GEMM workspace already held on "
            "this device.  The scratch is grow-only per (device, stream) -- see docs/API.md "
            "'Device memory' for the per-stream footprint; use fewer step streams or "
            "processes per GPU, or smaller products")


def dev_of(t: torch.Tensor) -> int:
    return 1 if t.is_cuda else 0


_raw_stream = getattr(torch._C, "_cuda_getCurrentRawStream", None)


def stream_of(t: torch.Tensor):
    if t.is_cuda:
        if _raw_stream is not None:
            return _raw_stream(t.get_device())
        return torch.cuda.current_stream(t.device).cuda_stream
    return None

# ... 40 lines not shown
```

moose_amd/ops/ring.py:

```python
from __future__ import annotations

import builtins
import ctypes
import functools
import math
import os
import threading
from fractions import Fraction
from typing import List
from typing import Sequence

import numpy as np
import torch

from moose_amd.ops import native as nat

MASK64 = (1 << 64) - 1
MASK128 = (1 << 128) - 1

_BIN = {"add": 0, "sub": 1, "mul": 2, "and": 3, "or": 4, "xor": 5}
_UN = {"neg": 0, "not": 1, "shl": 2, "shr": 3, "sar": 4}
_CMP = {"lt": 0, "gt": 1, "eq": 2, "msb": 3}


_UPLOAD_HOOK = None
_TLS = threading.local()


def upload_hook():
    h = getattr(_TLS, "hook", None)
    return h if h is not None else _UPLOAD_HOOK


def set_upload_hook(hook):
    prev = getattr(_TLS, "hook", None)
    _TLS.hook = hook
    return prev


def to_device(t: torch.Tensor, device) -> torch.Tensor:
    device = torch.device(device)
    if device.type == "cpu" or t.device == device:
        return t
    hook = upload_hook()
    if hook is not None:
        return hook(t, device)
    return t.to(device)


def _words(bits):
    return {1: 0, 64: 1, 128: 2}[bits]


class RT:

    __slots__ = ("data", "bits", "_shape")

    def __init__(self, data: torch.Tensor, bits: int):
        self.data = data
        self.bits = bits
        self._shape = None

    @property
    def shape(self):
        s = self._shape
        if s is None:
            s = tuple(self.data.shape)
            s = self._shape = s[:-1] if self.bits == 128 else s
        return s

    @property
    def ndim(self):
        return len(self.shape)

    @property
    def device(self):
        return self.data.device

    def numel(self):
        return math.prod(self.shape)

    def __repr__(self):
        return f"RT(bits={self.bits}, shape={self.shape}, device={self.device})"

    def contiguous(self):
        return RT(self.data.contiguous(), self.bits)

    def clone(self):
        return RT(self.data.clone(), self.bits)

# ... 1270 lines not shown

class PreparedCross:

    def __init__(self, y0: RT, y1: RT):
        self.y0, self.y1, self.bits = y0, y1, y0.bits
        self.batch, self.K, self.N = y0.shape[0], y0.shape[1], y0.shape[2]
        self.lb = None
        if y0.data.is_cuda:
            w = _words(self.bits)
            nbytes = nat.lib().mx_gemm_b_bytes(w, self.batch, self.N, self.K, 1)
            if nbytes > 0:
                d0, d1 = y0.data.contiguous(), y1.data.contiguous()
                self.lb = torch.empty(nbytes, dtype=torch.uint8, device=d0.device)
                nat.check(nat.lib().mx_gemm_prep_b(
                    w, self.batch, self.K, self.N, nat.ptr(d0), nat.ptr(d1), 1,
                    nat.ptr(self.lb), nat.stream_of(d0)), "gemm_prep_b")


def dot_cross_rows(x0: RT, x1: RT, r0: int, r1: int, pb: PreparedCross) -> RT:
    if pb.lb is None:
        rows = lambda t: RT(t.data[:, r0:r1], t.bits)
        return dot_cross(rows(x0), rows(x1), pb.y0, pb.y1, nb=1)
    batch, M, K = x0.shape
    d0, d1 = x0.data, x1.data
    if not (d0.is_contiguous() and d1.is_contiguous()):
        d0, d1 = d0.contiguous(), d1.contiguous()
    el = 2 if pb.bits == 128 else 1
    out = empty((batch, r1 - r0, pb.N), pb.bits, d0.device)
    off = r0 * K * el * 8
    nat.check(nat.lib().mx_gemm_with_b(
        _words(pb.bits), batch, r1 - r0, pb.N, K, ctypes.c_void_p(d0.data_ptr() + off),
        ctypes.c_void_p(d1.data_ptr() + off), M * K, 1,
        nat.ptr(pb.lb), nat.ptr(out.data), 0, nat.stream_of(d0)), "gemm_with_b")
    return out


def dot_cross_pair(x0: RT, y0: RT, y1: RT, roll: int, pb: PreparedCross = None, r0=0,
                   r1=None):
    d0 = x0.data
    if not d0.is_cuda or len(x0.shape) != 3:
        return None
    if not d0.is_contiguous():
        d0 = d0.contiguous()
    batch, M, K = x0.shape
    r1 = M if r1 is None else r1
    bits = x0.bits
    el = 2 if bits == 128 else 1
    if pb is not None:
        if pb.lb is None:
            return None
        N, lb, b0, b1 = pb.N, nat.ptr(pb.lb), None, None
    else:
        if (len(y0.shape) != 3 or tuple(y1.shape) != tuple(y0.shape)
                or y0.shape[0] != batch or y0.shape[1] != K):
            return None
        N = y0.shape[2]
        b0, b1 = y0.data.contiguous(), y1.data.contiguous()
        lb = None
    out = empty((batch, r1 - r0, N), bits, d0.device)
    rc = nat.lib().mx_gemm_roll(
        _words(bits), batch, r1 - r0, N, K, ctypes.c_void_p(d0.data_ptr() + r0 * K * el * 8),
        M * K, roll, None if b0 is None else nat.ptr(b0), None if b1 is None else nat.ptr(b1),
        lb, nat.ptr(out.data), 0, nat.stream_of(d0))
    if rc == -7:
        return None
    nat.check(rc, "gemm_roll")
    return out


def _asym_operands(x0: RT, x1: RT, y0: RT, y1: RT):
    def at(t, p):
        return RT(t.data[p], t.bits)

    a, b, c, d = ([at(t, p) for p in range(3)] for t in (x0, x1, y0, y1))
    zero = zeros(tuple(x0.shape[1:]), x0.bits, x0.device)
    stk = lambda ts: RT(torch.stack([t.data for t in ts]), x0.bits)
    A0 = stk([binary("add", a[0], b[0]), b[1], a[2]])
    A1 = stk([zero, a[1], b[2]])
    B0 = stk([c[0], d[1], c[2]])
    B1 = stk([d[0], c[1], binary("sub", d[2], c[2])])
    return A0, A1, B0, B1


def dot_cross_asym(x0: RT, x1: RT, y0: RT, y1: RT, rolled: bool = False) -> RT:
    bits = x0.bits
    M, K = x0.shape[1], x0.shape[2]
    N = y0.shape[2]
    d = x0.data
    if d.is_cuda and bits in (64, 128) and x0.shape[0] == 3 and y0.shape[0] == 3:
        ts = [t.data if t is not None else None for t in (x0, x1, y0, y1)]
        if rolled:
            ts[1] = ts[3] = None
        if all(t is None or t.is_contiguous() for t in ts):
            out = empty((3, M, N), bits, d.device)
            rc = nat.lib().mx_gemm_asym(
                _words(bits), M, N, K, nat.ptr(ts[0]), None if ts[1] is None else nat.ptr(ts[1]),
                nat.ptr(ts[2]), None if ts[3] is None else nat.ptr(ts[3]), 1 if rolled else 0,
                nat.ptr(out.data), nat.stream_of(d))
            if rc != -7:
                nat.check(rc, "gemm_asym")
                return out
    if x1 is None or y1 is None:
        x1 = RT(torch.roll(x0.data, -1, dims=0), bits)
        y1 = RT(torch.roll(y0.data, -1, dims=0), bits)
    A0, A1, B0, B1 = _asym_operands(x0, x1, y0, y1)
    return dot_cross(A0, A1, B0, B1, nb=1)


def dot_cross_asym_src(x0, y0, xsrc, ysrc, M: int, K: int, N: int):
    ts = [None if t is None else t.data for t in (x0, y0)]
    if any(t is not None and not t.is_contiguous() for t in ts):
        return None
    words = []
    for s in (xsrc, ysrc):
        if s is None:
            words.append(None)
            continue
        code, d, frac, j0, slot, nonce = s
        if not d.is_cuda or not d.is_contiguous():
            return None
        words.append((ctypes.c_int64 * 6)(d.data_ptr(), code, int(frac or 0), j0, int(slot),
                                          _i64(nonce)))
    anyt = next(s[1] for s in (xsrc, ysrc) if s is not None)
    out = empty((3, M, N), 128, anyt.device)
    rc = nat.lib().mx_gemm_asym_src(2, M, N, K, nat.ptr(ts[0]), nat.ptr(ts[1]), words[0],
                                    words[1], nat.ptr(out.data), nat.stream_of(anyt))
    if rc == -7:
        return None
    nat.check(rc, "gemm_asym_src")
    return out


def _i64(v: int) -> int:
    v &= (1 << 64) - 1
    return v - (1 << 64) if v >> 63 else v


def _party_batch_strides(t: RT):
    d = t.data
    el = 2 if t.bits == 128 else 1
    if d.dim() < 3:
        return None
    expect = 1
    for size, st in zip(reversed(d.shape[2:]), reversed(d.stride()[2:])):
        if size != 1 and st != expect:
            return None
        expect *= size
    if d.stride(0) % el or d.stride(1) % el:
        return None
    return d.stride(0) // el, d.stride(1) // el


def _dot_cross_strided(x0, x1, y0, y1, out, M, K, N):
    bits = x0.bits
    limit = (16384 if bits == 64 else 8192) // 2
    if not out.data.is_cuda or K > limit:
        return False
    st = [_party_batch_strides(t) for t in (x0, x1, y0, y1)]
    if any(s is None for s in st) or st[0][1] != st[1][1] or st[2][1] != st[3][1]:
        return False
    eb = 16 if bits == 128 else 8
    B = out.shape[1]
    lib = nat.lib()
    for p in range(out.shape[0]):
        def at(t, s):
            return ctypes.c_void_p(t.data.data_ptr() + p * s[0] * eb)
        optr = ctypes.c_void_p(out.data.data_ptr() + p * B * M * N * eb)
        nat.check(lib.mx_gemm_strided(_words(bits), B, M, N, K, at(x0, st[0]), at(x1, st[1]),
                                      st[0][1], at(y0, st[2]), at(y1, st[3]), st[2][1], 1, optr,
                                      0, nat.stream_of(out.data)), "gemm_strided")
    return True


def dot_cross(x0: RT, x1: RT, y0: RT, y1: RT, nb=0) -> RT:
    bits = x0.bits
    bshape, M, K, N, oshape = _dot_shapes(x0.shape, y0.shape, nb)
    batch = math.prod(bshape)
    out = empty(bshape + (M, N), bits, x0.device)
    if (nb == 2 and oshape == (M, N) and not all(
            t.data.is_contiguous() for t in (x0, x1, y0, y1))
            and _dot_cross_strided(x0, x1, y0, y1, out, M, K, N)):
        return out
    _gemm_call(
        bits, batch, M, N, K, x0.data.contiguous(), x1.data.contiguous(), y0.data.contiguous(),
        y1.data.contiguous(), 1, out.data,
    )
    return reshape(out, oshape, nb) if oshape != (M, N) else out


def prf_expand(keys: Sequence[bytes], nonce: int, shape, bits, device) -> RT:
    shape = tuple(shape)
    n = math.prod(shape)
    out = empty((len(keys),) + shape, bits, device)
    kb = nat.key_buffer(keys)
    if len(keys) > 4:
        raise ValueError("at most 4 keys per call")
    nat.check(
        nat.lib().mx_prf_expand(
            nat.dev_of(out.data), _words(bits), nat.ptr(out.data), n, len(keys), kb,
            nonce & MASK64, nat.stream_of(out.data),
        ),
        "prf_expand",
    )
    return out


def bit_planes(a: RT, start: int, count: int, nb=0) -> RT:
    shp = a.shape
    outer = math.prod(shp[:nb])
    inner = math.prod(shp[nb:])
    out = torch.empty(tuple(shp[:nb]) + (count,) + tuple(shp[nb:]), dtype=torch.uint8,
                      device=a.device)
    ad = a.data.contiguous()
# ... 265 lines not shown
def _mt3_args(x0: RT, x1: RT, y0: RT, y1: RT, out=None):
    bits = x0.bits
    if not x0.data.is_cuda or bits not in (64, 128):
        return None
    shp = x0.shape
    ops = (x0, x1, y0, y1)
    if any(o.shape != shp or o.bits != bits for o in ops):
        return None
    n = math.prod(shp) // 3
    if n == 0:
        return None
    views = None
    if any(not o.data.is_contiguous() for o in ops):
        vs = [_party_view(o) for o in ops]
        if any(v is None for v in vs):
            return None
        views = [v[0] for v in vs] + [v[1] for v in vs]
    w = 2 if bits == 128 else 1
    if out is None:
        o0, o1 = ring4(shp, bits, x0.device)
        os_ = n
    else:
        o0, o1 = out
        os_ = o0.data.stride(0) // w
        if not (o0.shape == shp and o1.shape == shp and o1.data.stride(0) == o0.data.stride(0)
                and o0.data[0].is_contiguous() and o1.data[0].is_contiguous()):
            return None
    return ops, (o0, o1), n, os_, views


def mul_trunc3_k2(jobs, slot_ptr: int):
    if len(jobs) != 2:
        return None
    prep = [_mt3_args(*j[:4], out=j[7]) for j in jobs]
    if any(p is None for p in prep) or jobs[0][0].bits != jobs[1][0].bits:
        return None
    bits = jobs[0][0].bits
    if any(p[2] > 8192 * (16 // (16 if bits == 128 else 8)) for p in prep):
        return None
    P2 = ctypes.c_void_p * 2
    ptr = lambda t: t.data.data_ptr()
    vws = [None if p[4] is None else (ctypes.c_int64 * 8)(*p[4]) for p in prep]
    views = (ctypes.c_void_p * 2)(*[None if v is None else ctypes.addressof(v) for v in vws])
    nn = (ctypes.c_uint64 * 12)(*[v & MASK64 for j in jobs for v in j[6]])
    rc = nat.lib().mxh_mul_trunc3_kv2(
        _words(bits), P2(*[ptr(p[0][0]) for p in prep]), P2(*[ptr(p[0][1]) for p in prep]),
        P2(*[ptr(p[0][2]) for p in prep]), P2(*[ptr(p[0][3]) for p in prep]),
        P2(*[ptr(p[1][0]) for p in prep]), P2(*[ptr(p[1][1]) for p in prep]),
        (ctypes.c_int64 * 2)(*[p[2] for p in prep]), (ctypes.c_int64 * 2)(*[p[3] for p in prep]),
        ctypes.c_void_p(slot_ptr), (ctypes.c_uint64 * 2)(*[j[4] & MASK64 for j in jobs]),
        (ctypes.c_int * 2)(*[int(j[5]) for j in jobs]), nn, views,
        nat.stream_of(jobs[0][0].data))
    if rc == -1:
        return None
    nat.check(rc, "mul_trunc3 x2")
    return [p[1] for p in prep]


def zs_trunc3_k(z: RT, slot_ptr: int, nmul: int, m: int, nonces):
    bits = z.bits
    if not z.data.is_cuda or bits not in (64, 128):
        return None
    d = z.data.contiguous()
    shp = z.shape
    n = math.prod(shp) // 3
    if n == 0:
        return None
    o0, o1 = ring4(shp, bits, d.device)
    nn = (ctypes.c_uint64 * 6)(*[v & MASK64 for v in nonces])
    rc = nat.lib().mx_mul_trunc3_kv(
        nat.dev_of(d), _words(bits), nat.ptr(d), None, None, None, nat.ptr(o0.data),
        nat.ptr(o1.data), n, n, ctypes.c_void_p(slot_ptr), nmul & MASK64, int(m), nn, None,
        nat.stream_of(d))
    if rc == 1:
        return None
    nat.check(rc, "zs_trunc3")
    return o0, o1


def zs_trunc3_open(z: RT, slot_ptr: int, nmul: int, m: int, nonces, frac: int):
    bits = z.bits
    if bits not in (64, 128):
        return None
    pv = _party_view(z)
    n = math.prod(z.shape) // 3
    if pv is None or pv[1] != n or pv[0] < n:
        d, xs = z.data.contiguous(), n
    else:
        d, xs = z.data, pv[0]
    if n == 0:
        return None
    out = torch.empty(z.shape[1:], dtype=torch.float64, device=d.device)
    nn = (ctypes.c_uint64 * 6)(*[v & MASK64 for v in nonces])
    nat.check(nat.lib().mx_mul_trunc3_open(
        nat.dev_of(d), _words(bits), nat.ptr(d), xs, nat.ptr(out), n, ctypes.c_void_p(slot_ptr),
        nmul & MASK64, int(m), nn, int(frac), nat.stream_of(d)), "zs_trunc3_open")
    return out


def zs_trunc3_rows(z: RT, slot_ptr: int, nmul: int, m: int, nonces, buf4, r0: int):
    bits = z.bits
    d = z.data.contiguous()
    n = math.prod(z.shape) // 3
    el = 2 if bits == 128 else 1
    os_ = math.prod(buf4.shape[1:]) // el
    o0 = buf4.data_ptr() + r0 * math.prod(buf4.shape[2:]) * 8
    nn = (ctypes.c_uint64 * 6)(*[v & MASK64 for v in nonces])
    rc = nat.lib().mx_mul_trunc3_kv(
        nat.dev_of(d), _words(bits), nat.ptr(d), None, None, None, ctypes.c_void_p(o0),
        ctypes.c_void_p(o0 + os_ * el * 8), n, os_, ctypes.c_void_p(slot_ptr), nmul & MASK64,
        int(m), nn, None, nat.stream_of(d))
    nat.check(rc, "zs_trunc3_rows")


def add_zs3(v: RT, r: RT):
    vd, rd = v.data.contiguous(), r.data.contiguous()
    n = math.prod(v.shape) // 3
    o0, o1 = empty(v.shape, v.bits, v.device), empty(v.shape, v.bits, v.device)
    nat.check(nat.lib().mx_add_zs3(nat.dev_of(vd), _words(v.bits), nat.ptr(vd), nat.ptr(rd),
                                   nat.ptr(o0.data), nat.ptr(o1.data), n, nat.stream_of(vd)),
              "add_zs3")
    return o0, o1


def _slot_operand_ok(a: RT, b: RT) -> bool:
    if b.numel() == 1:
        return True
    bs = list(b.shape)
    while bs and bs[0] == 1:
        bs.pop(0)
    ss = list(a.shape[1:])
    return len(bs) <= len(ss) and ss[len(ss) - len(bs):] == bs


def binary_slot(op: str, a: RT, b: RT, which: int):
    np_, m = a.shape[0], math.prod(a.shape[1:])
    nb = b.numel()
    if not _slot_operand_ok(a, b):
        raise ValueError("binary_slot: operand must be a scalar, one slot's shape or a "
                         "trailing-axes suffix of it")
    ad = a.data.contiguous()
    bd = b.data.contiguous()
    if bd.device != ad.device:
        bd = bd.to(ad.device)
    out = empty(a.shape, a.bits, a.device)
    nat.check(
        nat.lib().mx_ew_binary_slot(
            nat.dev_of(ad), _BIN[op], _words(a.bits), nat.ptr(ad), nat.ptr(bd), nb,
            nat.ptr(out.data), m, np_, int(which), nat.stream_of(ad),
        ),
        "binary_slot",
    )
    return out


def binary_slot2(op: str, a0: RT, a1: RT, b: RT, which0: int, which1: int):
    if a0.bits == 1 or a1.shape != a0.shape:
        return binary_slot(op, a0, b, which0), binary_slot(op, a1, b, which1)
    np_, m = a0.shape[0], math.prod(a0.shape[1:])
    nb = b.numel()
    if not _slot_operand_ok(a0, b):
        raise ValueError("binary_slot2: operand must be a scalar, one slot's shape or a "
                         "trailing-axes suffix of it")
    d0, d1, bd = a0.data.contiguous(), a1.data.contiguous(), b.data.contiguous()
    if bd.device != d0.device:
        bd = bd.to(d0.device)
    o0, o1 = empty2(a0.shape, a0.bits, a0.device)
    nat.check(nat.lib().mx_ew_binary_slot2(
        nat.dev_of(d0), _BIN[op], _words(a0.bits), nat.ptr(d0), nat.ptr(d1), nat.ptr(bd), nb,
        nat.ptr(o0.data), nat.ptr(o1.data), m, np_, int(which0), int(which1),
        nat.stream_of(d0)), "binary_slot (pair)")
    return o0, o1


_RT_DATA = RT.__dict__["data"]


class Opened(RT):

    __slots__ = ("parts", "stream")

    def __init__(self, a: RT, b: RT, c: RT, d: RT = None):
        _RT_DATA.__set__(self, None)
        self.bits = a.bits
        self._shape = a.shape
        self.parts = (a, b, c) if d is None else (a, b, c, d)
        self.stream = _stream_of(a.data)

    def pending(self) -> bool:
        return _RT_DATA.__get__(self) is None

    @property
    def data(self):
        d = _RT_DATA.__get__(self)
        if d is None:
            _join(self.stream)
            s = add3(*self.parts[:3])
            if len(self.parts) == 4:
                s = binary("add", s, self.parts[3])
            d = s.data
            _RT_DATA.__set__(self, d)
            self.parts = None
        return d

    @data.setter
    def data(self, v):
        _RT_DATA.__set__(self, v)

    @property
    def device(self):
        return self.parts[0].device if self.pending() else self.data.device


class OpenedTail(RT):

    __slots__ = ("src", "j")

    def __init__(self, src, j: int, shape):
        _RT_DATA.__set__(self, None)
        self.bits = src.bits
        self._shape = tuple(shape)
        self.src = src
        self.j = j

    def pending(self) -> bool:
        return _RT_DATA.__get__(self) is None

    def shares(self) -> RT:
        v0, v1 = self.src.s0.v, self.src.s1.v
        j, j1 = self.j, (self.j + 1) % 3
        return opened(RT(v0.data[j], v0.bits), RT(v1.data[j], v1.bits),
                      RT(v1.data[j1], v1.bits))

    @property
    def data(self):
        d = _RT_DATA.__get__(self)
        if d is None:
            d = self.shares().data
            _RT_DATA.__set__(self, d)
            self.src = None
        return d

    @data.setter
    def data(self, v):
        _RT_DATA.__set__(self, v)

    @property
    def device(self):
        return self.src.device if self.pending() else self.data.device


def opened(a: RT, b: RT, c: RT, d: RT = None) -> RT:
    parts = (a, b, c) if d is None else (a, b, c, d)
    if a.bits in (64, 128) and all(t.shape == a.shape and t.bits == a.bits for t in parts):
        return Opened(*parts)
    s = add3(a, b, c)
    return s if d is None else binary("add", s, d)


def add3(a: RT, b: RT, c: RT) -> RT:
    if not (a.shape == b.shape == c.shape and a.bits == b.bits == c.bits) or a.bits == 1:
        return binary("add", binary("add", a, b), c)
    d = [t.data.contiguous() for t in (a, b, c)]
    out = empty(a.shape, a.bits, a.device)
    nat.check(nat.lib().mx_ew_add3(nat.dev_of(d[0]), _words(a.bits), *[nat.ptr(x) for x in d],
                                   nat.ptr(out.data), a.numel(), nat.stream_of(d[0])), "add3")
    return out


def lincomb2(terms, b=None, which0: int = 0, which1: int = 2):
    c0, a0, _ = terms[0]
    bits, shp = a0.bits, a0.shape
    np_, m = shp[0], math.prod(shp[1:])
    datas = []
    for _, x0, x1 in terms:
        datas += [x0.data.contiguous(), x1.data.contiguous()]
    bd = None
    if b is not None:
        bd = b.data.contiguous()
        if bd.device != a0.device:
            bd = bd.to(a0.device)
    o0, o1 = empty2(shp, bits, a0.device)
    ins = (ctypes.c_void_p * len(datas))(*[d.data_ptr() for d in datas])
    coef = (ctypes.c_int64 * len(terms))(*[int(t[0]) for t in terms])
    nat.check(nat.lib().mx_lincomb2(
        nat.dev_of(o0.data), _words(bits), len(terms), ins, coef, nat.ptr(bd),
        b.numel() if b is not None else 0, nat.ptr(o0.data), nat.ptr(o1.data), m, np_,
        int(which0), int(which1), nat.stream_of(o0.data)), "lincomb2")
    return o0, o1


def _even_views(ts):
    d0 = ts[0].data
    w = 2 if ts[0].bits == 128 else 1
    if d0.dim() < 1 or not d0[0].is_contiguous() or d0.stride(0) % w:
        return None
    es = d0.element_size() * w
    ptrs = [t.data.data_ptr() for t in ts]
    for t in ts:
        d = t.data
        if (d.shape != d0.shape or d.stride() != d0.stride() or d.dtype != d0.dtype
                or d.device != d0.device or t.bits != ts[0].bits):
            return None
    if len(ts) > 1:
        step = ptrs[1] - ptrs[0]
        if step <= 0 or step % es or any(ptrs[i + 1] - ptrs[i] != step for i in range(len(ts) - 1)):
            return None
        step //= es
    else:
        step = 0
    return d0, step, d0.stride(0) // w


def sum_views2(ts0, ts1):
    v0, v1 = _even_views(ts0), _even_views(ts1)
    if v0 is None or v1 is None or ts0[0].shape != ts1[0].shape:
        return None
    bits, shp = ts0[0].bits, ts0[0].shape
    o0, o1 = empty2(shp, bits, ts0[0].device)
    np_, m = shp[0], math.prod(shp[1:])
    nat.check(nat.lib().mx_sum_views2(
        nat.dev_of(o0.data), _words(bits), v0[0].data_ptr(), v1[0].data_ptr(), v0[1], v1[1],
        v0[2], v1[2], len(ts0), nat.ptr(o0.data), nat.ptr(o1.data), m, np_,
        nat.stream_of(o0.data)), "sum_views2")
    return o0, o1


def b2a_prep3(b0: RT, b1: RT, ring_bits: int):
    d0, d1 = b0.data, b1.data
    if not d0.is_cuda or ring_bits not in (64, 128) or d0.dtype != torch.uint8 \
            or d1.dtype != torch.uint8 or d0.shape != d1.shape or d0.shape[0] != 3:
        return None
# ... 620 lines not shown
```

moose_amd/protocols/replicated.py:

```python
from __future__ import annotations

import os
from dataclasses import dataclass
from typing import Optional

import torch

from moose_amd.ir.computation import ReplicatedPlacement
from moose_amd.ops import ring as R
from moose_amd.runtime.session import HV
from moose_amd.runtime.session import PV
from moose_amd.runtime.session import Public
from moose_amd.utils.telemetry import span


@dataclass
class RepTensor:
    plc: ReplicatedPlacement
    bits: int
    kind: str
    s0: PV
    s1: PV
    zero_slot: Optional[int] = None

# ... 59 lines not shown
    def s1(self, v):
        self._s1 = v


_SCALED = {}


def _scaled_public(cv, m: int, bits: int):
    key = (id(cv), m, bits)
    hit = _SCALED.get(key)
    if hit is not None and hit[0] is cv:
        return hit[1]
    scaled = R.binary("mul", cv, R.fill((), 1 << m, bits, cv.data.device))
    capturing = cv.data.is_cuda and torch.cuda.is_current_stream_capturing()
    if len(_SCALED) < 1024 and not capturing and R.CONST_CACHE:
        _SCALED.setdefault(key, (cv, scaled))
    return scaled


class PendingTrunc(RepTensor):

    def __init__(self, sess, plc, bits, v_add, m, pubs=()):
        self._sess, self.v_add, self.m, self.pubs = sess, v_add, m, list(pubs)
        self.completed = False
        self._rb = None
        super().__init__(plc, bits, "arith", None, None)

    def with_public(self, c):
        return PendingTrunc(self._sess, self.plc, self.bits, self.v_add, self.m,
                            self.pubs + [c])

    def additive(self):
        v = self.v_add
        if self._sess.party_index(self.plc) == 0 and self.pubs:
            for c in self.pubs:
                v = R.binary("add", v, _scaled_public(c.v if isinstance(c, Public) else c,
                                                      self.m, self.bits))
        return v

    def _complete(self):
        if self.completed:
            if self._rb is not None:
                self._rb.finish()
            return
        self.completed = True
        sess, plc, bits = self._sess, self.plc, self.bits
        nonces = tuple(sess.nonce(plc) for _ in range(7))
        member = sess.party_index(plc) is not None
        v = self.additive() if member else self.v_add
        like = PV(plc, v)
        r = tail_job(sess, plc, bits, self.m, nonces, like,
                     lambda o0, o1: R.MulJob(1, o0, o1, a=v.data.contiguous()))
        self._s0, self._s1 = r.s0, r.s1

    def reshare_untruncated(self):
        sess, plc = self._sess, self.plc
        member = sess.party_index(plc) is not None
        z = sess.p_add_zero_share(plc, PV(plc, self.additive() if member else self.v_add))
        return _reshare(sess, plc, z, self.bits, "arith")

    @property
    def s0(self):
        self._complete()
        return self._s0

    @s0.setter
    def s0(self, v):
        self._s0 = v

    @property
    def s1(self):
        self._complete()
        return self._s1

    @s1.setter
    def s1(self, v):
        self._s1 = v


class StackedTail(RepTensor):

    def __init__(self, sess, plc, bits, v, m, nonces):
        self._sess, self.v, self.m, self._nonces = sess, v, m, nonces
        self._stream = R._stream_of(v.v.data)
        self.device = v.v.device
        super().__init__(plc, bits, "arith", None, None)

    @property
    def done(self) -> bool:
        return self._s0 is not None

    def finish(self):
        if self._s0 is None:
            R._join(self._stream)
            self._s0, self._s1 = self._sess.p_zs_trunc_run(self.plc, self.v, self.m,
                                                          self._nonces)
            self.v = None

    def open(self, frac: int):
        if self._s0 is not None:
            return None
        R._join(self._stream)
        return self._sess.p_zs_trunc_open(self.plc, self.v, self.m, self._nonces, frac)

    @property
    def s0(self):
        self.finish()
        return self._s0

    @s0.setter
    def s0(self, v):
        self._s0 = v

    @property
    def s1(self):
        self.finish()
        return self._s1

    @s1.setter
    def s1(self, v):
        self._s1 = v


class LazyShare(RepTensor):

    def __init__(self, sess, plc, bits, kind, issued, zero_slot):
        self._sess, self._issued = sess, issued
        self._stream = R._stream_of(issued[1])
        super().__init__(plc, bits, kind, None, None, zero_slot=zero_slot)

    @property
    def done(self) -> bool:
        return self._s0 is not None

    @property
    def shape(self):
        return tuple(self._issued[6])

    def source(self):
        return None if self.done else self._issued

    def finish(self):
        if self._s0 is None:
            R._join(self._stream)
            self._s0, self._s1 = self._sess.fused_share_run(self.plc, self._issued)
            self._issued = None

    @property
    def s0(self):
        self.finish()
        return self._s0

    @s0.setter
    def s0(self, v):
        self._s0 = v

    @property
    def s1(self):
        self.finish()
        return self._s1

    @s1.setter
    def s1(self, v):
        self._s1 = v


def lazy(x) -> bool:
# ... 458 lines not shown
    return "zero", "zero"


def _zero_slot_cross(sess, x: RepTensor, y: RepTensor):
    if not ZERO_SLOTS or x.zero_slot is None and y.zero_slot is None:
        return None
    xs0, xs1, ys0, ys1 = x.s0.v, x.s1.v, y.s0.v, y.s1.v
    if not all(isinstance(t, R.RT) for t in (xs0, xs1, ys0, ys1)):
        return None
    if len(xs0.shape) != 3 or len(ys0.shape) != 3 or x.bits not in (64, 128):
        return None
    terms = [_cross_terms(p, x.zero_slot, y.zero_slot) for p in range(3)]
    if any(t is None or t[0] == "zero" for t in terms):
        return None
    bits = x.bits

    def pick(name, s0, s1, p):
        a, b = R.RT(s0.data[p], bits), R.RT(s1.data[p], bits)
        return a if name[1:] == "0" else b if name[1:] == "1" else R.binary("add", a, b)

    A = torch.stack([pick(a, xs0, xs1, p).data for p, (a, _) in enumerate(terms)])
    B = torch.stack([pick(b, ys0, ys1, p).data for p, (_, b) in enumerate(terms)])
    return PV(x.plc, R.dot(R.RT(A, bits), R.RT(B, bits), nb=1))


def _dot_cross_src(sess, x: RepTensor, y: RepTensor):
    if not any(isinstance(t, LazyShare) and not t.done for t in (x, y)):
        return None
    fn = getattr(sess, "p_dot_cross_src", None)
    return fn(x.plc, x, y) if fn is not None else None


def dot(sess, x: RepTensor, y: RepTensor, nbatch: int = 0) -> RepTensor:
    with span("rep.dot"):
        over = getattr(sess, "p_dot_zs_reshare", None)
        if over is not None and getattr(sess, "fused", False) and not nbatch:
            res = over(x.plc, x.s0, x.s1, y.s0, y.s1, x.kind)
            if res is not None:
                return RepTensor(x.plc, x.bits, x.kind, res[0], res[1])
        if nbatch:
            v = sess.p_dot_cross(x.plc, x.s0, x.s1, y.s0, y.s1, nbatch=nbatch)
        else:
            v = _zero_slot_cross(sess, x, y) or sess.p_dot_cross(x.plc, x.s0, x.s1, y.s0,
                                                                    y.s1)
        fused = getattr(sess, "p_zero_share_reshare", None)
        if fused is not None and getattr(sess, "fused", False):
            s0, s1 = fused(x.plc, v, x.kind)
            return RepTensor(x.plc, x.bits, x.kind, s0, s1)
        z = sess.p_add_zero_share(x.plc, v, x.kind)
        return _reshare(sess, x.plc, z, x.bits, x.kind)


def _rows(pv: PV, r0: int, r1: int) -> PV:
    v = pv.v
    return PV(pv.plc, R.RT(v.data[:, r0:r1], v.bits))


def dot_trunc(sess, x: RepTensor, y: RepTensor, m: int, nbatch: int = 0) -> RepTensor:
    chunks = getattr(sess, "pipeline_chunks", 1)
    nchunk = 1
    if nbatch:
        if not (getattr(sess, "party_dot_trunc", None) is not None and m and 0 < m <= 63
                and x.kind == "arith" and x.bits in (64, 128)):
            return trunc_pr(sess, dot(sess, x, y, nbatch=nbatch), m)
        with span("rep.dot_trunc_party"):
            nonces = tuple(sess.nonce(x.plc) for _ in range(7))
            v = sess.p_dot_cross(x.plc, x.s0, x.s1, y.s0, y.s1, nbatch=nbatch)
            s0, s1 = sess.party_dot_trunc(x.plc, v, m, nonces)
            return RepTensor(x.plc, x.bits, "arith", s0, s1)
    if chunks > 1:
        xs, ys = x.s0.v.shape, y.s0.v.shape
        if len(xs) == 3 and len(ys) == 3:
            M = xs[1]
            nchunk = min(chunks, M // 128)
    party = getattr(sess, "party_dot_trunc", None)
    use_party = (party is not None and m and 0 < m <= 63 and x.kind == "arith"
                 and x.bits in (64, 128) and os.environ.get("MOOSEX_DOT_TAIL", "1") != "0")
    if nchunk <= 1:
        tail = getattr(sess, "p_zs_trunc", None)
        if (tail is not None and m and x.kind == "arith" and getattr(sess, "fused", False)
                and getattr(sess, "device", None) is not None and sess.device.type == "cuda"
                and os.environ.get("MOOSEX_DOT_TAIL", "1") != "0"):
            with span("rep.dot_trunc_fused"):
                v = (_zero_slot_cross(sess, x, y) or _dot_cross_src(sess, x, y)
                     or sess.p_dot_cross(x.plc, x.s0, x.s1, y.s0, y.s1))
                issue = getattr(sess, "p_zs_trunc_issue", None)
                if (issue is not None and x.bits in (64, 128)
                        and os.environ.get("MOOSEX_DOT_OPEN", "1") != "0"):
                    return StackedTail(sess, x.plc, x.bits, v, m, issue(x.plc, v))
                s0, s1 = tail(x.plc, v, m)
                return RepTensor(x.plc, x.bits, "arith", s0, s1)
        if use_party:
            with span("rep.dot_trunc_party"):
                nonces = tuple(sess.nonce(x.plc) for _ in range(7))
                pre_fn = getattr(sess, "party_dot_trunc_pre", None)
                pre = pre_fn(x.plc, x, y, m, nonces) if pre_fn is not None else None
                v = _zero_slot_cross(sess, x, y) or sess.p_dot_cross(x.plc, x.s0, x.s1, y.s0,
                                                                        y.s1)
                if getattr(sess, "defer_reshare", False) and pre is not None:
                    s0, s1, rb = party(x.plc, v, m, nonces, pre=pre, defer=True)
                    return DeferredRep(x.plc, x.bits, "arith", s0, s1, rb)
                s0, s1 = (party(x.plc, v, m, nonces) if pre is None
                          else party(x.plc, v, m, nonces, pre=pre))
                return RepTensor(x.plc, x.bits, "arith", s0, s1)
        return trunc_pr(sess, dot(sess, x, y), m)
    with span("rep.dot_trunc_pipelined"):
        plc, bits, kind = x.plc, x.bits, x.kind
        bounds = [M * c // nchunk for c in range(nchunk + 1)]
        data = x.s0.v.data
        cuda = data.is_cuda
        main = torch.cuda.current_stream(data.device) if cuda else None
        side = sess.side_stream() if cuda else None
        prepared = sess.p_prepare_cross(plc, y.s0, y.s1)
        N = y.s0.v.shape[2]
        shp = (3, M, N) + ((2,) if bits == 128 else ())
        rows_fused = (cuda and getattr(sess, "fused", False) and m and kind == "arith"
                      and bits in (64, 128) and getattr(sess, "p_zs_trunc_rows", None) is not None)
        if rows_fused:
            buf4 = torch.empty((4,) + shp[1:], dtype=data.dtype, device=data.device)
            out0, out1 = buf4[0:3], buf4[1:4]
        else:
            out0 = torch.empty(shp, dtype=data.dtype, device=data.device)
            out1 = torch.empty_like(out0)

        def tail(v, r0, r1):
            if rows_fused:
                sess.p_zs_trunc_rows(plc, v, m, buf4, r0)
                return
            if use_party:
                nonces = tuple(sess.nonce(plc) for _ in range(7))
                party(plc, v, m, nonces, out=(out0[:, r0:r1], out1[:, r0:r1]))
                return
            z = sess.p_add_zero_share(plc, v, kind)
            t = trunc_pr(sess, _reshare(sess, plc, z, bits, kind), m)
            out0[:, r0:r1].copy_(t.s0.v.data)
            out1[:, r0:r1].copy_(t.s1.v.data)

        for c in range(nchunk):
            r0, r1 = bounds[c], bounds[c + 1]
            v = sess.p_dot_cross_rows(plc, x.s0, x.s1, r0, r1, prepared)
            if not cuda:
                tail(v, r0, r1)
                continue
            ev = torch.cuda.Event()
            ev.record(main)
            with torch.cuda.stream(side):
                side.wait_event(ev)
                v.v.data.record_stream(side)
                tail(v, r0, r1)
        if cuda:
            main.wait_stream(side)
        return RepTensor(plc, bits, kind, PV(plc, R.RT(out0, bits)), PV(plc, R.RT(out1, bits)))


def dwconv_trunc(sess, x: RepTensor, w: RepTensor, m: int, geom: dict) -> RepTensor:
    tail = getattr(sess, "p_zs_trunc", None)
    if (tail is not None and m and x.kind == "arith" and getattr(sess, "fused", False)
            and getattr(sess, "device", None) is not None and sess.device.type == "cuda"
            and os.environ.get("MOOSEX_DOT_TAIL", "1") != "0"):
        with span("rep.dwconv_trunc_fused"):
            v = sess.p_dwconv_cross(x.plc, x.s0, x.s1, w.s0, w.s1, geom)
            issue = getattr(sess, "p_zs_trunc_issue", None)
            if (issue is not None and x.bits in (64, 128)
                    and os.environ.get("MOOSEX_DOT_OPEN", "1") != "0"):
                return StackedTail(sess, x.plc, x.bits, v, m, issue(x.plc, v))
            s0, s1 = tail(x.plc, v, m)
            return RepTensor(x.plc, x.bits, "arith", s0, s1)
    party = getattr(sess, "party_dot_trunc", None)
    if (party is not None and m and 0 < m <= 63 and x.kind == "arith" and x.bits in (64, 128)
            and os.environ.get("MOOSEX_DOT_TAIL", "1") != "0"):
        with span("rep.dwconv_trunc_party"):
# ... 372 lines not shown
```

Baseline: 1.513 billion.

## Defer CRT reconstruction and fuse it into the truncation-open kernel

The GEMM can now return the raw multi-modular residues as a lazy CrtProduct, so reconstruction back into ring elements no longer runs unconditionally. When the product is opened straight after a fused dot-trunc, a new kernel rebuilds the three party products from the residues, adds the PRF masks, applies the truncation and writes doubles in one pass. This removes the write and reread of the (3,M,N) 128-bit intermediate. The cost is that the residue tensor stays alive longer, the PRF work is duplicated per strip, and the fused kernel reconstructs all three shares per lane serially, which may lower parallelism.

```diff
diff --git a/csrc/gemm_crt.hip b/csrc/gemm_crt.hip
--- a/csrc/gemm_crt.hip
+++ b/csrc/gemm_crt.hip
@@ -1103,13 +1103,66 @@
   }
 }
 
+template <class T>
+__device__ __forceinline__ void recon16d_lane(const int8_t* __restrict__ src, int64_t pstride,
+                                              int n, const RecTab4& r4, const RecTab& rc,
+                                              T (&z)[4]) {
+  constexpr int ND = (int)sizeof(T);
+  constexpr int NK = ND / 2;
+  int acc[4][ND], aq[4][3];
+#pragma unroll
+  for (int e = 0; e < 4; ++e) {
+#pragma unroll
+    for (int d = 0; d < ND; ++d) acc[e][d] = 0;
+#pragma unroll
+    for (int d = 0; d < 3; ++d) aq[e][d] = 0;
+  }
+  for (int g = 0; g < r4.groups; ++g) {
+    uint32_t v[4];
+#pragma unroll
+    for (int u = 0; u < 4; ++u)
+      v[u] = 4 * g + u < n ? *(const uint32_t*)(src + (4 * g + u) * pstride) : 0u;
+    const uint32_t a0 = __builtin_amdgcn_perm(v[1], v[0], 0x05010400u);
+    const uint32_t a1 = __builtin_amdgcn_perm(v[1], v[0], 0x07030602u);
+    const uint32_t c0 = __builtin_amdgcn_perm(v[3], v[2], 0x05010400u);
+    const uint32_t c1 = __builtin_amdgcn_perm(v[3], v[2], 0x07030602u);
+    const int t[4] = {(int)__builtin_amdgcn_perm(c0, a0, 0x05040100u),
+                      (int)__builtin_amdgcn_perm(c0, a0, 0x07060302u),
+                      (int)__builtin_amdgcn_perm(c1, a1, 0x05040100u),
+                      (int)__builtin_amdgcn_perm(c1, a1, 0x07060302u)};
+#pragma unroll
+    for (int d = 0; d < ND; ++d) {
+      const int w = (int)r4.wd[g][d];
+#pragma unroll
+      for (int e = 0; e < 4; ++e) acc[e][d] = __builtin_amdgcn_sdot4(t[e], w, acc[e][d], false);
+    }
+#pragma unroll
+    for (int d = 0; d < 3; ++d) {
+      const int w = (int)r4.rd[g][d];
+#pragma unroll
+      for (int e = 0; e < 4; ++e) aq[e][d] = __builtin_amdgcn_sdot4(t[e], w, aq[e][d], false);
+    }
+  }
+  T mw = 0;
+#pragma unroll
+  for (int k = 0; k < NK; ++k) mw |= (T)rc.Mw[k] << (16 * k);
+#pragma unroll
+  for (int e = 0; e < 4; ++e) {
+    T s = 0;
+#pragma unroll
+    for (int k = 0; k < NK; ++k)
+      s += (T)(int64_t)(acc[e][2 * k] + acc[e][2 * k + 1] * 256) << (16 * k);
+    const int64_t F = (int64_t)aq[e][0] + (int64_t)aq[e][1] * 256 + (int64_t)aq[e][2] * 65536;
+    const int64_t q = (F + (1 << 23)) >> 24;
+    z[e] = s - (T)q * mw;
+  }
+}
+
 template <class T, int BN>
 __global__ void __launch_bounds__(256)
     k_crt_recon16d(const int8_t* __restrict__ CR, T* __restrict__ C, int64_t M, int64_t N,
                    int64_t tiles_m, int64_t tiles_n, int accumulate, const RecTab4 r4, int n,
                    const RecTab rc) {
-  constexpr int ND = (int)sizeof(T);
-  constexpr int NK = ND / 2;
   constexpr int kCrTile = BM * BN, NBJ = BN / 16;
   const int64_t ntiles = tiles_m * tiles_n;
   const int64_t total = ntiles * (kCrTile / 4);
@@ -1121,63 +1174,86 @@
     const int blk = (int)(rest % (16 * NBJ));
     const int64_t tile = rest / (16 * NBJ);
     const int64_t off = tile * kCrTile + (blk * 64 + lane) * 4;
-    int acc[4][ND], aq[4][3];
-#pragma unroll
-    for (int e = 0; e < 4; ++e) {
-#pragma unroll
-      for (int d = 0; d < ND; ++d) acc[e][d] = 0;
-#pragma unroll
-      for (int d = 0; d < 3; ++d) aq[e][d] = 0;
-    }
-    const int8_t* src = CR + b * n * ntiles * (int64_t)kCrTile + off;
     const int64_t pstride = ntiles * (int64_t)kCrTile;
-    for (int g = 0; g < r4.groups; ++g) {
-      uint32_t v[4];
-#pragma unroll
-      for (int u = 0; u < 4; ++u)
-        v[u] = 4 * g + u < n ? *(const uint32_t*)(src + (4 * g + u) * pstride) : 0u;
-      const uint32_t a0 = __builtin_amdgcn_perm(v[1], v[0], 0x05010400u);
-      const uint32_t a1 = __builtin_amdgcn_perm(v[1], v[0], 0x07030602u);
-      const uint32_t c0 = __builtin_amdgcn_perm(v[3], v[2], 0x05010400u);
-      const uint32_t c1 = __builtin_amdgcn_perm(v[3], v[2], 0x07030602u);
-      const int t[4] = {(int)__builtin_amdgcn_perm(c0, a0, 0x05040100u),
-                        (int)__builtin_amdgcn_perm(c0, a0, 0x07060302u),
-                        (int)__builtin_amdgcn_perm(c1, a1, 0x05040100u),
-                        (int)__builtin_amdgcn_perm(c1, a1, 0x07060302u)};
-#pragma unroll
-      for (int d = 0; d < ND; ++d) {
-        const int w = (int)r4.wd[g][d];
-#pragma unroll
-        for (int e = 0; e < 4; ++e) acc[e][d] = __builtin_amdgcn_sdot4(t[e], w, acc[e][d], false);
-      }
-#pragma unroll
-      for (int d = 0; d < 3; ++d) {
-        const int w = (int)r4.rd[g][d];
-#pragma unroll
-        for (int e = 0; e < 4; ++e) aq[e][d] = __builtin_amdgcn_sdot4(t[e], w, aq[e][d], false);
-      }
-    }
+    T z[4];
+    recon16d_lane<T>(CR + b * n * pstride + off, pstride, n, r4, rc, z);
     const int64_t tm = tile / tiles_n, tn = tile % tiles_n;
     const int bi = blk / NBJ, bj = blk % NBJ;
     const int64_t gcol = tn * BN + bj * 16 + (lane & 15);
-    T mw = 0;
-#pragma unroll
-    for (int k = 0; k < NK; ++k) mw |= (T)rc.Mw[k] << (16 * k);
 #pragma unroll
     for (int e = 0; e < 4; ++e) {
       const int64_t grow = tm * BM + bi * 16 + 4 * (lane >> 4) + e;
-      T z = 0;
-#pragma unroll
-      for (int k = 0; k < NK; ++k)
-        z += (T)(int64_t)(acc[e][2 * k] + acc[e][2 * k + 1] * 256) << (16 * k);
-      const int64_t F = (int64_t)aq[e][0] + (int64_t)aq[e][1] * 256 + (int64_t)aq[e][2] * 65536;
-      const int64_t q = (F + (1 << 23)) >> 24;
-      z -= (T)q * mw;
       if (grow < M && gcol < N) {
         T* pc = C + (b * M + grow) * N + gcol;
-        *pc = accumulate ? (T)(*pc + z) : z;
-      }
-    }
+        *pc = accumulate ? (T)(*pc + z[e]) : z[e];
+      }
+    }
+  }
+}
+
+template <class T>
+__global__ void __launch_bounds__(256)
+    k_crt_recon16d_open(const int8_t* __restrict__ CR, double* __restrict__ out, double scale,
+                        int64_t M, int64_t N, int64_t tiles_n, int64_t pstride,
+                        const RecTab4 r4, int n, const RecTab rc, mxd::KeySrc keys, uint64_t nr0,
+                        uint64_t nr1, int m) {
+  constexpr int BN = 256, kCrTile = BM * BN, P = mxd::Lane<T>::kPer;
+  __shared__ uint32_t rks[3][mxd::kKeyWords];
+  __shared__ T rr[8][BN];
+  mxd::stage_keys(rks, keys, 3);
+  const int tid = threadIdx.x, wave = tid >> 6, lane = tid & 63;
+  const int64_t strips = ((M + 7) / 8) * tiles_n;
+  for (int64_t s = blockIdx.x; s < strips; s += gridDim.x) {
+    const int64_t row0 = (s / tiles_n) * 8, tn = s % tiles_n, col0 = tn * BN;
+    const int64_t ncol = N - col0 < BN ? N - col0 : BN;
+    for (int i = wave; i < 8; i += 4) {
+      if (row0 + i >= M) break;
+      const int64_t f0 = (row0 + i) * N + col0, f1 = f0 + ncol;
+      for (int64_t G = (f0 / P) >> 8; G <= ((f1 - 1) / P) >> 8; ++G) {
+        const uint64_t B = ((uint64_t)G << 6) | (uint64_t)lane;
+        uint32_t w0[16], w1[16];
+        mx::chacha_block(rks[0], nr0, B, w0);
+        mx::chacha_block(rks[2], nr1, B, w1);
+#pragma unroll
+        for (int part = 0; part < 4; ++part) {
+          const int64_t c = (int64_t)mx::ks_chunk(B, part);
+          uint64_t lo0, hi0, lo1, hi1;
+          mx::part_u64(w0, part, &lo0, &hi0);
+          mx::part_u64(w1, part, &lo1, &hi1);
+#pragma unroll
+          for (int j = 0; j < P; ++j) {
+            const int64_t e = c * P + j;
+            if (e >= f0 && e < f1)
+              rr[i][e - f0] = mxd::pick<T>(lo0, hi0, j) + mxd::pick<T>(lo1, hi1, j);
+          }
+        }
+      }
+    }
+    __syncthreads();
+    const int q = (tid >> 4) & 1;
+    const int64_t grow0 = row0 + 4 * q;
+    const int64_t tile = (grow0 / BM) * tiles_n + tn;
+    const int bi = (int)(grow0 % BM) / 16, l16 = ((int)(grow0 % 16) / 4) * 16 + (tid & 15);
+#pragma unroll 1
+    for (int h = 0; h < 2; ++h) {
+      const int ct = h * 128 + (tid >> 5) * 16 + (tid & 15);
+      if (grow0 >= M || ct >= ncol) continue;
+      const int64_t off = tile * kCrTile + ((bi * (BN / 16) + ct / 16) * 64 + l16) * 4;
+      T x[4] = {0, 0, 0, 0};
+#pragma unroll 1
+      for (int b = 0; b < 3; ++b) {
+        T z[4];
+        recon16d_lane<T>(CR + b * n * pstride + off, pstride, n, r4, rc, z);
+#pragma unroll
+        for (int e = 0; e < 4; ++e) x[e] += z[e];
+      }
+#pragma unroll
+      for (int e = 0; e < 4; ++e)
+        if (grow0 + e < M)
+          out[(grow0 + e) * N + col0 + ct] =
+              mxr::signed_to_f64<T>(mxf::trunc_pr_open<T>(x[e], rr[4 * q + e][ct], m)) * scale;
+    }
+    __syncthreads();
   }
 }
 
@@ -1395,6 +1471,26 @@
                        M, N, p.tiles_m, p.tiles_n, accumulate, tb.rc);
 }
 
+bool defer_ok(const CPlan& p) { return p.bn == 256 && crt_mfma16() && recon_dot4() && p.n > 0; }
+
+CPlan asym_plan(int words, int64_t M, int64_t N, int64_t K) {
+  CPlan p;
+  p.n = -1;
+  if ((words != 1 && words != 2) || K % BK || !crt_mfma16() || 2 * K > (1 << 15)) return p;
+  return make_cplan(words, 3, M, N, K, 1, true);
+}
+
+template <class T>
+void launch_recon_open(const CPlan& p, const Tables& tb, int64_t M, int64_t N, const int8_t* cr,
+                       double* out, double scale, const mxd::KeySrc& keys, uint64_t nr0,
+                       uint64_t nr1, int m, hipStream_t st) {
+  const int64_t strips = ((M + 7) / 8) * p.tiles_n;
+  const int64_t pstride = p.tiles_m * p.tiles_n * (int64_t)(BM * 256);
+  hipLaunchKernelGGL((k_crt_recon16d_open<T>), dim3((unsigned)std::min<int64_t>(strips, 1 << 20)),
+                     dim3(256), 0, st, cr, out, scale, M, N, p.tiles_n, pstride, tb.r4, p.n,
+                     tb.rc, keys, nr0, nr1, m);
+}
+
 struct Ws {
   void* ptr = nullptr;
   int64_t bytes = 0;
@@ -1477,7 +1573,7 @@
 template <class T>
 int run_crt_asym(int64_t M, int64_t N, int64_t K, const T* S0, const T* S1, const T* T0,
                  const T* T1, int rolled, T* C, hipStream_t st, const ShareSrc* xs = nullptr,
-                 const ShareSrc* ys = nullptr) {
+                 const ShareSrc* ys = nullptr, int8_t* cr_ext = nullptr) {
   constexpr int words = sizeof(T) / 8;
   if (K % BK || !crt_mfma16()) return -7;
   if (2 * K > (1 << 15)) return -6;
@@ -1547,12 +1643,13 @@
   if (ys) plan_src(true, *ys, bph, bat, nb, bmap, b_strip);
   const int64_t ra_bytes = na * a_entry, rb_bytes = nb * b_entry;
   const int64_t sum_bytes = asum && !duals ? round_up(sa * (int64_t)sizeof(T), 256) : 0;
-  int8_t* ws = (int8_t*)workspace(
-      a_strip + ra_bytes + p.cr_bytes + b_strip + rb_bytes + sum_bytes, st);
+  if (cr_ext && !defer_ok(p)) return -7;
+  const int64_t cr_ws = cr_ext ? 0 : p.cr_bytes;
+  int8_t* ws = (int8_t*)workspace(a_strip + ra_bytes + cr_ws + b_strip + rb_bytes + sum_bytes, st);
   if (!ws) return -4;
   int8_t* ra = ws + a_strip;
-  int8_t* cr = ra + ra_bytes;
-  int8_t* rb = cr + p.cr_bytes + b_strip;
+  int8_t* cr = cr_ext ? cr_ext : ra + ra_bytes;
+  int8_t* rb = ra + ra_bytes + cr_ws + b_strip;
   T* a01 = sum_bytes ? (T*)(rb + rb_bytes) : nullptr;
   if (a01)
     hipLaunchKernelGGL((k_add_pair<T>), dim3((unsigned)std::min<int64_t>((sa + 255) / 256, 65536)),
@@ -1600,7 +1697,7 @@
     launch_prep<T>(p, tb, false, sa_.n, M, K, 0, nullptr, nullptr, 0, ra, st, kn, kn, sa_);
   }
   launch_crt_gemm(p, tb, 3, ra, rb, cr, 0, 0, st, amap, bmap);
-  launch_recon<T>(p, tb, 3, M, N, cr, C, 0, st);
+  if (!cr_ext) launch_recon<T>(p, tb, 3, M, N, cr, C, 0, st);
   const hipError_t e = hipGetLastError();
   return e != hipSuccess ? -100 - (int)e : 0;
 }
@@ -1610,22 +1707,67 @@
 extern "C" {
 
 int mx_gemm_asym(int words, int64_t M, int64_t N, int64_t K, const void* S0, const void* S1,
-                 const void* T0, const void* T1, int rolled, void* C, void* stream) {
-  if (M == 0 || N == 0) return 0;
+                 const void* T0, const void* T1, int rolled, void* C, void* stream,
+                 void* residues) {
+  if (M == 0 || N == 0) return residues ? -7 : 0;
   if (!rolled && (!S1 || !T1)) return -2;
   hipStream_t st = (hipStream_t)stream;
   if (words == 1)
     return run_crt_asym<u64>(M, N, K, (const u64*)S0, (const u64*)S1, (const u64*)T0,
-                             (const u64*)T1, rolled, (u64*)C, st);
+                             (const u64*)T1, rolled, (u64*)C, st, nullptr, nullptr,
+                             (int8_t*)residues);
   if (words == 2)
     return run_crt_asym<u128>(M, N, K, (const u128*)S0, (const u128*)S1, (const u128*)T0,
-                              (const u128*)T1, rolled, (u128*)C, st);
+                              (const u128*)T1, rolled, (u128*)C, st, nullptr, nullptr,
+                              (int8_t*)residues);
   return -2;
 }
 
+int64_t mx_crt_defer_bytes(int words, int64_t M, int64_t N, int64_t K) {
+  if (M <= 0 || N <= 0) return -7;
+  const CPlan p = asym_plan(words, M, N, K);
+  return p.n > 0 && defer_ok(p) ? p.cr_bytes : -7;
+}
+
+int mx_crt_recon(int words, int64_t M, int64_t N, int64_t K, const void* residues, void* C,
+                 void* stream) {
+  const CPlan p = asym_plan(words, M, N, K);
+  if (p.n <= 0 || !defer_ok(p)) return -7;
+  const Tables& tb = tables_for(words, p.n);
+  hipStream_t st = (hipStream_t)stream;
+  if (words == 1)
+    launch_recon<u64>(p, tb, 3, M, N, (const int8_t*)residues, (u64*)C, 0, st);
+  else
+    launch_recon<u128>(p, tb, 3, M, N, (const int8_t*)residues, (u128*)C, 0, st);
+  const hipError_t e = hipGetLastError();
+  return e != hipSuccess ? -100 - (int)e : 0;
+}
+
+int mxh_crt_recon_open(int words, const int64_t* crt, double* out, int64_t n,
+                       const uint32_t* slots, int m, const uint64_t* nn, int frac, void* stream) {
+  const int64_t M = crt[1], N = crt[2], K = crt[3];
+  if (M <= 0 || N <= 0 || n != M * N || !crt[0]) return -3;
+  const CPlan p = asym_plan(words, M, N, K);
+  if (p.n <= 0 || !defer_ok(p)) return -7;
+  const Tables& tb = tables_for(words, p.n);
+  const uint32_t* ptrs[3];
+  for (int i = 0; i < 3; ++i) ptrs[i] = slots + MX_KEY_SLOT_WORDS * i;
+  const mxd::KeySrc keys = mxd::keysrc_slots(ptrs, 3);
+  const int8_t* cr = (const int8_t*)(intptr_t)crt[0];
+  const double scale = std::ldexp(1.0, -frac);
+  hipStream_t st = (hipStream_t)stream;
+  if (words == 1)
+    launch_recon_open<u64>(p, tb, M, N, cr, out, scale, keys, nn[0], nn[1], m, st);
+  else
+    launch_recon_open<u128>(p, tb, M, N, cr, out, scale, keys, nn[0], nn[1], m, st);
+  const hipError_t e = hipGetLastError();
+  return e != hipSuccess ? -100 - (int)e : 0;
+}
+
 int mx_gemm_asym_src(int words, int64_t M, int64_t N, int64_t K, const void* S0, const void* T0,
-                     const int64_t* xsrc, const int64_t* ysrc, void* C, void* stream) {
-  if (M == 0 || N == 0) return 0;
+                     const int64_t* xsrc, const int64_t* ysrc, void* C, void* stream,
+                     void* residues) {
+  if (M == 0 || N == 0) return residues ? -7 : 0;
   if (words != 2) return -7;
   if ((!xsrc && !S0) || (!ysrc && !T0)) return -2;
   ShareSrc sx, sy;
@@ -1643,7 +1785,7 @@
   if ((xsrc && !sx.key.slot[0]) || (ysrc && !sy.key.slot[0])) return -2;
   return run_crt_asym<u128>(M, N, K, (const u128*)S0, nullptr, (const u128*)T0, nullptr, 1,
                             (u128*)C, (hipStream_t)stream, xsrc ? &sx : nullptr,
-                            ysrc ? &sy : nullptr);
+                            ysrc ? &sy : nullptr, (int8_t*)residues);
 }
 
 int mx_crt_moduli(int words, int64_t kprime) {
diff --git a/csrc/moosex.h b/csrc/moosex.h
--- a/csrc/moosex.h
+++ b/csrc/moosex.h
@@ -67,7 +67,7 @@
                      const int64_t* views, void* stream);
 int mx_mul_trunc3_open(int dev, int words, const void* x, int64_t xstride, double* out,
                        int64_t n, const uint32_t* slots, uint64_t nmul, int m,
-                       const uint64_t* nonces, int frac, void* stream);
+                       const uint64_t* nonces, int frac, void* stream, const int64_t* crt);
 int mx_ew_add3(int dev, int words, const void* a, const void* b, const void* c, void* out,
                int64_t n, void* stream);
 int mx_lincomb2(int dev, int words, int nin, const void* const* ins, const int64_t* coef,
diff --git a/csrc/ring_common.h b/csrc/ring_common.h
--- a/csrc/ring_common.h
+++ b/csrc/ring_common.h
@@ -170,6 +170,14 @@
     r = (double)top * p;
   }
   return neg ? -r : r;
+}
+
+template <class T>
+MX_HD inline double signed_to_f64(T v) {
+  if constexpr (sizeof(T) == 8)
+    return (double)(int64_t)v;
+  else
+    return i128_to_f64(v);
 }
 
 }
@@ -240,6 +248,8 @@
 int mxh_mul_trunc3_open(int words, const void* x, int64_t xstride, double* out, int64_t n,
                         const uint32_t* slots, uint64_t nmul, int m, const uint64_t* nn, int frac,
                         void* stream);
+int mxh_crt_recon_open(int words, const int64_t* crt, double* out, int64_t n,
+                       const uint32_t* slots, int m, const uint64_t* nn, int frac, void* stream);
 int mxh_ew_unary2(int op, int words, const void* a0, void* out0, const void* a1, void* out1,
                   int64_t n, int64_t param, void* stream);
 int mxh_transpose2(int words, const void* a0, void* out0, const void* a1, void* out1,
diff --git a/csrc/ring_hip.hip b/csrc/ring_hip.hip
--- a/csrc/ring_hip.hip
+++ b/csrc/ring_hip.hip
@@ -1414,11 +1414,7 @@
   double* __restrict__ out;
   double scale;
   __device__ __forceinline__ void operator()(int64_t e, T Z0, T Z1, T Z2) const {
-    const T v = Z0 + Z1 + Z2;
-    if constexpr (sizeof(T) == 8)
-      out[e] = (double)(int64_t)v * scale;
-    else
-      out[e] = mxr::i128_to_f64(v) * scale;
+    out[e] = mxr::signed_to_f64<T>(Z0 + Z1 + Z2) * scale;
   }
 };
 
diff --git a/csrc/rss_fused.h b/csrc/rss_fused.h
--- a/csrc/rss_fused.h
+++ b/csrc/rss_fused.h
@@ -37,6 +37,19 @@
   T ov1 = rm1 - shl<T>(c_msb * rm1, 1);
   T y1 = shl<T>(ov1, k - m) - rt1;
   return (y0 - z0) + (y1 - z2);
+}
+
+template <class T>
+MX_HD inline T trunc_pr_open(T x, T r, int m) {
+  constexpr int W = 8 * sizeof(T);
+  const int k = W - 1;
+  T r_msb = shr<T>(r, W - 1);
+  T r_top = shr<T>(shl<T>(r, 1), m + 1);
+  T c = x + shl<T>((T)1, k - 1) + r;
+  T c_msb = shr<T>(c, W - 1);
+  T c_top = shr<T>(shl<T>(c, 1), m + 1);
+  T ov = r_msb - shl<T>(c_msb * r_msb, 1) + c_msb;
+  return shl<T>(ov, k - m) - r_top + c_top - shl<T>((T)1, k - 1 - m);
 }
 
 template <class T>
diff --git a/csrc/rss_fused_cpu.cpp b/csrc/rss_fused_cpu.cpp
--- a/csrc/rss_fused_cpu.cpp
+++ b/csrc/rss_fused_cpu.cpp
@@ -250,9 +250,11 @@
 
 int mx_mul_trunc3_open(int dev, int words, const void* x, int64_t xstride, double* out,
                        int64_t n, const uint32_t* slots, uint64_t nmul, int m,
-                       const uint64_t* nonces, int frac, void* stream) {
+                       const uint64_t* nonces, int frac, void* stream, const int64_t* crt) {
   if (words != 1 && words != 2) return -2;
   if (m < 1 || m > 63) return -3;
+  if (crt)
+    return dev ? mxh_crt_recon_open(words, crt, out, n, slots, m, nonces, frac, stream) : -2;
   if (dev) return mxh_mul_trunc3_open(words, x, xstride, out, n, slots, nmul, m, nonces, frac,
                                       stream);
   if (xstride < n) return -3;
diff --git a/moose_amd/ops/native.py b/moose_amd/ops/native.py
--- a/moose_amd/ops/native.py
+++ b/moose_amd/ops/native.py
@@ -41,7 +41,7 @@
     "mx_mul_trunc3_kv": (c_int, [c_int, c_int, c_vp, c_vp, c_vp, c_vp, c_vp, c_vp, c_i64, c_i64,
                                  c_vp, c_u64, c_int, c_vp, c_vp, c_vp]),
     "mx_mul_trunc3_open": (c_int, [c_int, c_int, c_vp, c_i64, c_vp, c_i64, c_vp, c_u64, c_int,
-                                   c_vp, c_int, c_vp]),
+                                   c_vp, c_int, c_vp, c_vp]),
     "mx_ew_add3": (c_int, [c_int, c_int, c_vp, c_vp, c_vp, c_vp, c_i64, c_vp]),
     "mx_lincomb2": (c_int, [c_int, c_int, c_int, c_vp, c_vp, c_vp, c_i64, c_vp, c_vp, c_i64,
                             c_int, c_int, c_int, c_vp]),
@@ -268,11 +268,13 @@
     "mx_copy_many": (c_int, [c_vp, c_int, c_i64, c_vp]),
     "mx_graph_free": (c_int, [c_vp, c_vp]),
     "mx_gemm_asym": (
-        c_int, [c_int, c_i64, c_i64, c_i64, c_vp, c_vp, c_vp, c_vp, c_int, c_vp, c_vp],
+        c_int, [c_int, c_i64, c_i64, c_i64, c_vp, c_vp, c_vp, c_vp, c_int, c_vp, c_vp, c_vp],
     ),
     "mx_gemm_asym_src": (
-        c_int, [c_int, c_i64, c_i64, c_i64, c_vp, c_vp, c_vp, c_vp, c_vp, c_vp],
-    ),
+        c_int, [c_int, c_i64, c_i64, c_i64, c_vp, c_vp, c_vp, c_vp, c_vp, c_vp, c_vp],
+    ),
+    "mx_crt_defer_bytes": (c_i64, [c_int, c_i64, c_i64, c_i64]),
+    "mx_crt_recon": (c_int, [c_int, c_i64, c_i64, c_i64, c_vp, c_vp, c_vp]),
     "mx_gemm_roll": (
         c_int,
         [c_int, c_i64, c_i64, c_i64, c_i64, c_vp, c_i64, c_i64, c_vp, c_vp, c_vp, c_vp, c_int,
diff --git a/moose_amd/ops/ring.py b/moose_amd/ops/ring.py
--- a/moose_amd/ops/ring.py
+++ b/moose_amd/ops/ring.py
@@ -6,6 +6,7 @@
 import math
 import os
 import threading
+from contextlib import contextmanager
 from fractions import Fraction
 from typing import List
 from typing import Sequence
@@ -1442,6 +1443,28 @@
     return A0, A1, B0, B1
 
 
+_DEFER = threading.local()
+
+
+@contextmanager
+def deferred_products(on: bool = True):
+    prev = getattr(_DEFER, "on", False)
+    _DEFER.on = bool(on)
+    try:
+        yield
+    finally:
+        _DEFER.on = prev
+
+
+def _defer_residues(bits: int, M: int, N: int, K: int, device):
+    if not getattr(_DEFER, "on", False):
+        return None
+    nbytes = nat.lib().mx_crt_defer_bytes(_words(bits), M, N, K)
+    if nbytes < 0:
+        return None
+    return torch.empty(nbytes, dtype=torch.int8, device=device)
+
+
 def dot_cross_asym(x0: RT, x1: RT, y0: RT, y1: RT, rolled: bool = False) -> RT:
     bits = x0.bits
     M, K = x0.shape[1], x0.shape[2]
@@ -1452,14 +1475,15 @@
         if rolled:
             ts[1] = ts[3] = None
         if all(t is None or t.is_contiguous() for t in ts):
-            out = empty((3, M, N), bits, d.device)
+            res = _defer_residues(bits, M, N, K, d.device)
+            out = empty((3, M, N), bits, d.device) if res is None else None
             rc = nat.lib().mx_gemm_asym(
                 _words(bits), M, N, K, nat.ptr(ts[0]), None if ts[1] is None else nat.ptr(ts[1]),
                 nat.ptr(ts[2]), None if ts[3] is None else nat.ptr(ts[3]), 1 if rolled else 0,
-                nat.ptr(out.data), nat.stream_of(d))
+                None if out is None else nat.ptr(out.data), nat.stream_of(d), nat.ptr(res))
             if rc != -7:
                 nat.check(rc, "gemm_asym")
-                return out
+                return out if res is None else CrtProduct(res, M, N, K, bits)
     if x1 is None or y1 is None:
         x1 = RT(torch.roll(x0.data, -1, dims=0), bits)
         y1 = RT(torch.roll(y0.data, -1, dims=0), bits)
@@ -1482,13 +1506,15 @@
         words.append((ctypes.c_int64 * 6)(d.data_ptr(), code, int(frac or 0), j0, int(slot),
                                           _i64(nonce)))
     anyt = next(s[1] for s in (xsrc, ysrc) if s is not None)
-    out = empty((3, M, N), 128, anyt.device)
+    res = _defer_residues(128, M, N, K, anyt.device)
+    out = empty((3, M, N), 128, anyt.device) if res is None else None
     rc = nat.lib().mx_gemm_asym_src(2, M, N, K, nat.ptr(ts[0]), nat.ptr(ts[1]), words[0],
-                                    words[1], nat.ptr(out.data), nat.stream_of(anyt))
+                                    words[1], None if out is None else nat.ptr(out.data),
+                                    nat.stream_of(anyt), nat.ptr(res))
     if rc == -7:
         return None
     nat.check(rc, "gemm_asym_src")
-    return out
+    return out if res is None else CrtProduct(res, M, N, K, 128)
 
 
 def _i64(v: int) -> int:
@@ -1920,6 +1946,8 @@
     bits = z.bits
     if bits not in (64, 128):
         return None
+    if isinstance(z, CrtProduct) and z.pending():
+        return z.open(slot_ptr, nmul, m, nonces, frac)
     pv = _party_view(z)
     n = math.prod(z.shape) // 3
     if pv is None or pv[1] != n or pv[0] < n:
@@ -1932,7 +1960,7 @@
     nn = (ctypes.c_uint64 * 6)(*[v & MASK64 for v in nonces])
     nat.check(nat.lib().mx_mul_trunc3_open(
         nat.dev_of(d), _words(bits), nat.ptr(d), xs, nat.ptr(out), n, ctypes.c_void_p(slot_ptr),
-        nmul & MASK64, int(m), nn, int(frac), nat.stream_of(d)), "zs_trunc3_open")
+        nmul & MASK64, int(m), nn, int(frac), nat.stream_of(d), None), "zs_trunc3_open")
     return out
 
 
@@ -2086,6 +2114,62 @@
     @property
     def device(self):
         return self.src.device if self.pending() else self.data.device
+
+
+class CrtProduct(RT):
+
+    __slots__ = ("residues", "mnk", "stream")
+
+    def __init__(self, residues: torch.Tensor, M: int, N: int, K: int, bits: int):
+        _RT_DATA.__set__(self, None)
+        self.bits = bits
+        self._shape = (3, M, N)
+        self.residues = residues
+        self.mnk = (M, N, K)
+        self.stream = _stream_of(residues)
+
+    def pending(self) -> bool:
+        return _RT_DATA.__get__(self) is None
+
+    def _residues_here(self) -> torch.Tensor:
+        _join(self.stream)
+        cur = torch.cuda.current_stream(self.residues.device)
+        if cur != self.stream:
+            self.residues.record_stream(cur)
+        return self.residues
+
+    def open(self, slot_ptr: int, nmul: int, m: int, nonces, frac: int) -> torch.Tensor:
+        res = self._residues_here()
+        M, N, K = self.mnk
+        out = torch.empty((M, N), dtype=torch.float64, device=res.device)
+        nn = (ctypes.c_uint64 * 6)(*[v & MASK64 for v in nonces])
+        crt = (ctypes.c_int64 * 4)(res.data_ptr(), M, N, K)
+        nat.check(nat.lib().mx_mul_trunc3_open(
+            1, _words(self.bits), None, 0, nat.ptr(out), M * N, ctypes.c_void_p(slot_ptr),
+            nmul & MASK64, int(m), nn, int(frac), nat.stream_of(res), crt), "zs_trunc3_open (crt)")
+        return out
+
+    @property
+    def data(self):
+        d = _RT_DATA.__get__(self)
+        if d is None:
+            res = self._residues_here()
+            M, N, K = self.mnk
+            out = empty((3, M, N), self.bits, res.device)
+            nat.check(nat.lib().mx_crt_recon(_words(self.bits), M, N, K, nat.ptr(res),
+                                             nat.ptr(out.data), nat.stream_of(res)), "crt_recon")
+            d = out.data
+            _RT_DATA.__set__(self, d)
+            self.residues = None
+        return d
+
+    @data.setter
+    def data(self, v):
+        _RT_DATA.__set__(self, v)
+
+    @property
+    def device(self):
+        return self.residues.device if self.pending() else self.data.device
 
 
 def opened(a: RT, b: RT, c: RT, d: RT = None) -> RT:
diff --git a/moose_amd/protocols/replicated.py b/moose_amd/protocols/replicated.py
--- a/moose_amd/protocols/replicated.py
+++ b/moose_amd/protocols/replicated.py
@@ -165,7 +165,8 @@
 
     def __init__(self, sess, plc, bits, v, m, nonces):
         self._sess, self.v, self.m, self._nonces = sess, v, m, nonces
-        self._stream = R._stream_of(v.v.data)
+        lazy_v = isinstance(v.v, R.CrtProduct) and v.v.pending()
+        self._stream = v.v.stream if lazy_v else R._stream_of(v.v.data)
         self.device = v.v.device
         super().__init__(plc, bits, "arith", None, None)
 
@@ -790,11 +791,14 @@
                 and getattr(sess, "device", None) is not None and sess.device.type == "cuda"
                 and os.environ.get("MOOSEX_DOT_TAIL", "1") != "0"):
             with span("rep.dot_trunc_fused"):
-                v = (_zero_slot_cross(sess, x, y) or _dot_cross_src(sess, x, y)
-                     or sess.p_dot_cross(x.plc, x.s0, x.s1, y.s0, y.s1))
                 issue = getattr(sess, "p_zs_trunc_issue", None)
-                if (issue is not None and x.bits in (64, 128)
-                        and os.environ.get("MOOSEX_DOT_OPEN", "1") != "0"):
+                waits = (issue is not None and x.bits in (64, 128)
+                         and os.environ.get("MOOSEX_DOT_OPEN", "1") != "0")
+                with R.deferred_products(
+                        waits and os.environ.get("MOOSEX_DOT_OPEN_FUSED", "1") != "0"):
+                    v = (_zero_slot_cross(sess, x, y) or _dot_cross_src(sess, x, y)
+                         or sess.p_dot_cross(x.plc, x.s0, x.s1, y.s0, y.s1))
+                if waits:
                     return StackedTail(sess, x.plc, x.bits, v, m, issue(x.plc, v))
                 s0, s1 = tail(x.plc, v, m)
                 return RepTensor(x.plc, x.bits, "arith", s0, s1)
```

New measurement: 1.576 billion (median of 6 runs). +4.2%, better.
